# ZPP-Robotics/OSQP-Solver

Hardware: AMD Instinct MI355X
Metric: QPs/sec on a 1024-QP batch of box-QPs (n=512, m=1024), OSQP defaults; ADMM iters/sec alongside (higher is better)
Workload: dtype f64

## Files before the change

### include/mi_osqp.h

```cpp
#ifndef MI_OSQP_H
#define MI_OSQP_H

#include <stdint.h>

#ifdef __cplusplus
extern "C" {
#endif

typedef enum {
  MI_OSQP_OK = 0,
  MI_OSQP_ERR_INVALID_DATA = 1,
  MI_OSQP_ERR_INVALID_SETTINGS = 2,
  MI_OSQP_ERR_PATTERN_CHANGED = 3,
  MI_OSQP_ERR_NONCONVEX = 4,
  MI_OSQP_ERR_DEVICE = 5,
  MI_OSQP_ERR_NULL = 6,
  MI_OSQP_ERR_ALLOC = 7
} mi_osqp_error;

typedef enum {
  MI_OSQP_EXIT_OPTIMAL = 0,
  MI_OSQP_EXIT_PRIMAL_INFEASIBLE = 1,
  MI_OSQP_EXIT_DUAL_INFEASIBLE = 2,
  MI_OSQP_EXIT_OPTIMAL_INACCURATE = 3,
  MI_OSQP_EXIT_PRIMAL_INFEASIBLE_INACCURATE = 4,
  MI_OSQP_EXIT_DUAL_INFEASIBLE_INACCURATE = 5,
  MI_OSQP_EXIT_MAX_ITERATIONS = 6,
  MI_OSQP_EXIT_INTERRUPTED = 7,
  MI_OSQP_EXIT_TIME_LIMIT_REACHED = 8,
  MI_OSQP_EXIT_NON_CONVEX = 9,
  MI_OSQP_EXIT_UNKNOWN = 10
} mi_osqp_exit_code;

typedef struct {
  double  rho;
  double  sigma;
  int64_t scaling;
  int64_t adaptive_rho;
  int64_t adaptive_rho_interval;
  double  adaptive_rho_tolerance;
  int64_t max_iter;
  double  eps_abs;
  double  eps_rel;
  double  eps_prim_inf;
  double  eps_dual_inf;
  double  alpha;
  int64_t scaled_termination;
  int64_t check_termination;
  int64_t warm_start;
  int64_t verbose;
  int64_t polish;
  int64_t polish_refine_iter;
  double  delta;
} mi_osqp_settings;

typedef struct {
  int64_t iter;
  int64_t status_val;
  int64_t exit_code;
  double  obj_val;
  double  pri_res;
  double  dua_res;
  int64_t rho_updates;
  double  rho_estimate;
  double  rho;
  int64_t status_polish;
} mi_osqp_info;

typedef struct {
  int64_t n, m, N, batch, tile, n_tiles;
  int64_t nnz_P_triu, nnz_A, nnz_KKT, nnz_L;
  int64_t n_supernodes, n_blocks;
  int64_t fwd_levels, bwd_levels, fwd_slots, bwd_slots, chk_slots;
  int64_t lds_bytes, threads_per_block;
  int64_t dense_tail_rows, dense_tail_slots;
  double  setup_seconds_host, setup_seconds_factor, setup_seconds_upload;
  int64_t nnz_L_before_tail;
  int64_t solve_groups, solve_group_threads;
  int64_t resident_state, lds_bytes_iterate;
  int64_t pipelined_refactors;
  int64_t resident_factor_steps, lds_bytes_factor;
  int64_t dense_tail_tasks, dense_tail_waves_used, dense_tail_wave_tasks_max;
  int64_t refactor_lanes;
  int64_t iterate_launches_deep_ring, iterate_launches_long_head;
  int64_t runahead_regions, runahead_tiles, runahead_left, runahead_missed;
} mi_osqp_stats;

typedef struct mi_osqp_solver mi_osqp_solver;
typedef struct mi_osqp_batch  mi_osqp_batch;

void        mi_osqp_default_settings(mi_osqp_settings *s);
const char *mi_osqp_exit_code_name(int64_t exit_code);
const char *mi_osqp_error_name(int64_t err);
const char *mi_osqp_version(void);
const char *mi_osqp_last_error(void);

int mi_osqp_setup(mi_osqp_solver **out, int64_t n, int64_t m,
                  const int64_t *P_colptr, const int64_t *P_rowidx, const double *P_val,
                  const double *q,
                  const int64_t *A_colptr, const int64_t *A_rowidx, const double *A_val,
                  const double *l, const double *u, const mi_osqp_settings *settings);
int mi_osqp_update_A(mi_osqp_solver *h, const int64_t *A_colptr, const int64_t *A_rowidx,
                     const double *A_val);
int mi_osqp_update_bounds(mi_osqp_solver *h, const double *l, const double *u);
int mi_osqp_update_A_bounds(mi_osqp_solver *h, const int64_t *A_colptr, const int64_t *A_rowidx, const double *A_val,
                            const double *l, const double *u);
int mi_osqp_warm_start_x(mi_osqp_solver *h, const double *x);
int mi_osqp_update_q(mi_osqp_solver *h, const double *q);
int mi_osqp_update_P(mi_osqp_solver *h, const int64_t *P_colptr, const int64_t *P_rowidx, const double *P_val);
int mi_osqp_update_P_A(mi_osqp_solver *h, const int64_t *P_colptr, const int64_t *P_rowidx, const double *P_val,
                       const int64_t *A_colptr, const int64_t *A_rowidx, const double *A_val);
int mi_osqp_warm_start_y(mi_osqp_solver *h, const double *y);
int mi_osqp_solve(mi_osqp_solver *h, mi_osqp_info *info);
int mi_osqp_get_primal(mi_osqp_solver *h, double *x_out);
int mi_osqp_get_dual(mi_osqp_solver *h, double *y_out);
int mi_osqp_get_prim_inf_cert(mi_osqp_solver *h, double *dy_out );
int mi_osqp_get_dual_inf_cert(mi_osqp_solver *h, double *dx_out );
int mi_osqp_adjoint(mi_osqp_solver *h, const double *dx, const double *dy, double *dq, double *dP, double *dA, double *dl, double *du,
                    int32_t *status);
int mi_osqp_get_stats(mi_osqp_solver *h, mi_osqp_stats *st);
int mi_osqp_get_settings(mi_osqp_solver *h, mi_osqp_settings *out);
int mi_osqp_update_settings(mi_osqp_solver *h, const mi_osqp_settings *s);
void mi_osqp_free(mi_osqp_solver *h);

int mi_osqp_batch_setup(mi_osqp_batch **out, int64_t B, int64_t n, int64_t m,
                        const int64_t *P_colptr, const int64_t *P_rowidx, const double *P_val,
                        const double *q,
                        const int64_t *A_colptr, const int64_t *A_rowidx, const double *A_val,
                        const double *l, const double *u, const mi_osqp_settings *settings,
                        int64_t device);
int mi_osqp_batch_update_A(mi_osqp_batch *h, const int64_t *A_colptr, const int64_t *A_rowidx,
                           const double *A_val);
int mi_osqp_batch_update_bounds(mi_osqp_batch *h, const double *l, const double *u);
int mi_osqp_batch_update_A_bounds(mi_osqp_batch *h, const int64_t *A_colptr, const int64_t *A_rowidx, const double *A_val,
                                  const double *l, const double *u);
int mi_osqp_batch_warm_start_x(mi_osqp_batch *h, const double *x);
int mi_osqp_batch_update_q(mi_osqp_batch *h, const double *q);
int mi_osqp_batch_update_P(mi_osqp_batch *h, const int64_t *P_colptr, const int64_t *P_rowidx, const double *P_val);
int mi_osqp_batch_update_P_A(mi_osqp_batch *h, const int64_t *P_colptr, const int64_t *P_rowidx, const double *P_val,
                             const int64_t *A_colptr, const int64_t *A_rowidx, const double *A_val);
int mi_osqp_batch_warm_start_y(mi_osqp_batch *h, const double *y);
int mi_osqp_batch_get_P_upper_pattern(mi_osqp_batch *h, int64_t *colptr, int64_t *rowidx, int64_t *nnz_out);
int mi_osqp_batch_solve(mi_osqp_batch *h);
int mi_osqp_batch_get_primal(mi_osqp_batch *h, double *x_out );
int mi_osqp_batch_get_dual(mi_osqp_batch *h, double *y_out );
int mi_osqp_batch_get_info(mi_osqp_batch *h, mi_osqp_info *info );
int mi_osqp_batch_get_prim_inf_cert(mi_osqp_batch *h, double *dy_out );
int mi_osqp_batch_get_dual_inf_cert(mi_osqp_batch *h, double *dx_out );
int mi_osqp_batch_get_stats(mi_osqp_batch *h, mi_osqp_stats *st);
int mi_osqp_batch_get_ordering(mi_osqp_batch *h, int64_t *kkt_perm);
void mi_osqp_batch_free(mi_osqp_batch *h);
int mi_osqp_prefetch_analysis(int64_t B, int64_t n, int64_t m, const int64_t *Pp, const int64_t *Pi,
                              const int64_t *Ap, const int64_t *Ai, int64_t device);
void mi_osqp_release_device_cache(void);

int mi_osqp_batch_update_bounds_device(mi_osqp_batch *h, const double *d_l, const double *d_u, void *stream);
int mi_osqp_batch_update_A_bounds_device(mi_osqp_batch *h, const double *d_Av, const double *d_l, const double *d_u, void *stream);
int mi_osqp_batch_update_q_device(mi_osqp_batch *h, const double *d_q, void *stream);
int mi_osqp_batch_update_P_device(mi_osqp_batch *h, const double *d_Pv, void *stream);
int mi_osqp_batch_update_P_A_bounds_device(mi_osqp_batch *h, const double *d_Pv, const double *d_Av, const double *d_l, const double *d_u,
                                           void *stream);
int mi_osqp_batch_solve_device(mi_osqp_batch *h, double *d_x_out, int32_t *d_status, int32_t *d_iters, void *stream);
int mi_osqp_batch_reset(mi_osqp_batch *h);
int mi_osqp_batch_last_solve_stats(mi_osqp_batch *h, int64_t *total_iters, int64_t *kernel_launches,
                                   double *device_seconds, double *refactor_seconds, int64_t *refactor_count,
                                   double *compact_seconds);
int mi_osqp_batch_last_polish_stats(mi_osqp_batch *h, int64_t *polished, int64_t *accepted, double *seconds);
int mi_osqp_batch_get_polish_active(mi_osqp_batch *h, int8_t *act);
// ... 40 lines not shown
  MI_GOMP_MODEL_DH_CHAIN = 6
} mi_gomp_model;
typedef struct { int32_t model; int32_t is_gripper; double radius; double param[12]; } mi_gomp_ball;
typedef struct { double dir[2]; double point[3]; int32_t below; int32_t reserved; } mi_gomp_line;
typedef struct mi_gomp_scene mi_gomp_scene;
int mi_gomp_scene_create(mi_gomp_scene **out, mi_osqp_batch *h, int64_t dims, int64_t waypoints,
                         int64_t n_balls, const mi_gomp_ball *balls, int64_t n_lines, const mi_gomp_line *lines,
                         const double *con_lo, const double *con_hi);
typedef struct { int32_t n_joints; int32_t reserved; double a[8], d[8], alpha[8], theta0[8]; } mi_gomp_chain;
int mi_gomp_scene_create_chain(mi_gomp_scene **out, mi_osqp_batch *h, int64_t dims, int64_t waypoints,
                               const mi_gomp_chain *chain, int64_t n_balls, const mi_gomp_ball *balls,
                               int64_t n_lines, const mi_gomp_line *lines, const double *con_lo, const double *con_hi);
typedef struct { double a[3], b[3]; double radius; double margin; } mi_gomp_capsule;
int mi_gomp_scene_create_world(mi_gomp_scene **out, mi_osqp_batch *h, int64_t dims, int64_t waypoints,
                               const mi_gomp_chain *chain, int64_t n_balls, const mi_gomp_ball *balls,
                               int64_t n_lines, const mi_gomp_line *lines, int64_t n_capsules, const mi_gomp_capsule *capsules,
                               const double *con_lo, const double *con_hi);
void mi_gomp_scene_free(mi_gomp_scene *sc);
int mi_gomp_scene_set_rows(mi_gomp_scene *sc, int64_t n_ids, const int64_t *ids, const double *A_val, const double *l, const double *u);
int mi_gomp_scene_get_rows(mi_gomp_scene *sc, int64_t id, double *A_val, double *l, double *u);
int mi_gomp_assemble_some(mi_gomp_scene *sc, int64_t n_ids, const int64_t *ids, const double *x, int32_t *ok_out);
int mi_gomp_relinearise_some(mi_gomp_scene *sc, int64_t n_ids, const int64_t *ids, const double *x, int32_t *ok_out);

typedef struct mi_osqp_multi mi_osqp_multi;
int mi_osqp_multi_batch_setup(mi_osqp_multi **out, int64_t n_devices, const int64_t *devices,
                              int64_t B, int64_t n, int64_t m,
                              const int64_t *P_colptr, const int64_t *P_rowidx, const double *P_val,
                              const double *q,
                              const int64_t *A_colptr, const int64_t *A_rowidx, const double *A_val,
                              const double *l, const double *u, const mi_osqp_settings *settings);
int mi_osqp_multi_batch_update_A(mi_osqp_multi *h, const int64_t *A_colptr, const int64_t *A_rowidx, const double *A_val);
int mi_osqp_multi_batch_update_bounds(mi_osqp_multi *h, const double *l, const double *u);
int mi_osqp_multi_batch_update_A_bounds(mi_osqp_multi *h, const int64_t *A_colptr, const int64_t *A_rowidx, const double *A_val,
                                        const double *l, const double *u);
int mi_osqp_multi_batch_warm_start_x(mi_osqp_multi *h, const double *x);
int mi_osqp_multi_batch_update_q(mi_osqp_multi *h, const double *q);
int mi_osqp_multi_batch_update_P(mi_osqp_multi *h, const int64_t *P_colptr, const int64_t *P_rowidx, const double *P_val);
int mi_osqp_multi_batch_update_P_A(mi_osqp_multi *h, const int64_t *P_colptr, const int64_t *P_rowidx, const double *P_val,
                                   const int64_t *A_colptr, const int64_t *A_rowidx, const double *A_val);
int mi_osqp_multi_batch_warm_start_y(mi_osqp_multi *h, const double *y);
int mi_osqp_multi_batch_get_settings(mi_osqp_multi *h, mi_osqp_settings *out);
int mi_osqp_multi_batch_update_settings(mi_osqp_multi *h, const mi_osqp_settings *s);
int mi_osqp_multi_batch_update_rho_each(mi_osqp_multi *h, const double *rho );
int mi_osqp_multi_batch_solve(mi_osqp_multi *h);
int mi_osqp_multi_batch_solve_async(mi_osqp_multi *h);
int mi_osqp_multi_batch_wait(mi_osqp_multi *h);
int mi_osqp_multi_batch_get_primal(mi_osqp_multi *h, double *x_out );
int mi_osqp_multi_batch_get_dual(mi_osqp_multi *h, double *y_out );
int mi_osqp_multi_batch_get_info(mi_osqp_multi *h, mi_osqp_info *info );
int mi_osqp_multi_batch_get_prim_inf_cert(mi_osqp_multi *h, double *dy_out );
int mi_osqp_multi_batch_get_dual_inf_cert(mi_osqp_multi *h, double *dx_out );
int64_t mi_osqp_multi_batch_shards(mi_osqp_multi *h);
int mi_osqp_multi_batch_shard(mi_osqp_multi *h, int64_t k, int64_t *device, int64_t *begin, int64_t *end, mi_osqp_batch **handle);
void mi_osqp_multi_batch_free(mi_osqp_multi *h);

int mi_osqp_batch_spmv(mi_osqp_batch *h, const double *d_x, const double *d_y,
                       double *d_Px, double *d_Aty, double *d_Ax, void *stream);
int mi_osqp_batch_kkt_solve(mi_osqp_batch *h, const double *d_rhs, double *d_sol, void *stream);
int mi_osqp_batch_refactor_device(mi_osqp_batch *h);
int mi_osqp_batch_kernel_time(mi_osqp_batch *h, double *avg_ms, int64_t *launches);
int mi_osqp_batch_refactor_time(mi_osqp_batch *h, double *factor_ms, double *tail_ms, int64_t *launches, int64_t *qps);
int mi_osqp_batch_refactor_peak(mi_osqp_batch *h, int64_t *qps, double *factor_ms, double *tail_ms);

int mi_osqp_batch_get_scaling(mi_osqp_batch *h, double *D , double *E , double *c );

int mi_osqp_debug_host_kkt_solve(int64_t n, int64_t m,
                                 const int64_t *P_colptr, const int64_t *P_rowidx, const double *P_val,
                                 const int64_t *A_colptr, const int64_t *A_rowidx, const double *A_val,
                                 const double *l, const double *u, const mi_osqp_settings *settings,
                                 int64_t tile, const double *rhs ,
                                 double *sol_schedule , double *sol_direct ,
                                 mi_osqp_stats *st);

int mi_osqp_debug_host_block_factor(int64_t n, int64_t m,
                                    const int64_t *P_colptr, const int64_t *P_rowidx, const double *P_val,
                                    const int64_t *A_colptr, const int64_t *A_rowidx, const double *A_val,
                                    const double *l, const double *u, const mi_osqp_settings *settings,
                                    double *max_rel_diff_L, double *max_rel_diff_Dinv, int64_t *counts);

int mi_osqp_debug_refactor_chunks(int64_t n_flagged, const int64_t *flagged, int64_t n_active, const int64_t *active, int64_t tile,
                                  int64_t chunk_qps, int64_t max_chunks, int64_t *n_chunks, int64_t *work_begin, int64_t *tiles,
                                  int64_t *tile_begin);

int mi_osqp_debug_refactor_lanes(int64_t n_flagged, const int64_t *flagged, int64_t n_active, const int64_t *active, int64_t tile,
                                 int64_t chunk_qps, int64_t max_chunks, int64_t kbt, int64_t lanes, int64_t chunk0_first,
                                 int64_t scratch_slots, int64_t *n_lanes, int64_t *lane_of, int64_t *order, int64_t *order_begin,
                                 int64_t *scratch_begin, int64_t *n_waits, int64_t *wait_chunk, int64_t *wait_for);

int mi_osqp_debug_runahead_group(int64_t n_active, const int64_t *tiles, const double *pri_res, const double *dua_res, int64_t size,
                                 int64_t min_active, int64_t *n_group, int64_t *group);

int mi_osqp_debug_iterate_form(int64_t tiles, int64_t has_head, int64_t forced_form, int64_t long_min, int64_t *form);

int mi_osqp_debug_trace_kkt_solve(mi_osqp_batch *h, int32_t which, const double *d_rhs, double *d_sol,
                                  uint32_t *out, int64_t out_capacity_words, int64_t *dims);

#ifdef __cplusplus
}
#endif
#endif
```

### osqp-solver_amd/__init__.py

```python
import ctypes as C
import os

import numpy as np

try:
    import torch
except ImportError:
    torch = None

from . import build as _build

_HERE = os.path.dirname(os.path.abspath(__file__))
_LIB = None

EXIT_NAMES = ["kOptimal", "kPrimalInfeasible", "kDualInfeasible", "kOptimalInaccurate",
              "kPrimalInfeasibleInaccurate", "kDualInfeasibleInaccurate", "kMaxIterations",
              "kInterrupted", "kTimeLimitReached", "kNonConvex", "kUnknown"]
K_OPTIMAL = 0


class Settings(C.Structure):
    _fields_ = [("rho", C.c_double), ("sigma", C.c_double), ("scaling", C.c_int64),
                ("adaptive_rho", C.c_int64), ("adaptive_rho_interval", C.c_int64),
                ("adaptive_rho_tolerance", C.c_double), ("max_iter", C.c_int64),
                ("eps_abs", C.c_double), ("eps_rel", C.c_double), ("eps_prim_inf", C.c_double),
                ("eps_dual_inf", C.c_double), ("alpha", C.c_double), ("scaled_termination", C.c_int64),
                ("check_termination", C.c_int64), ("warm_start", C.c_int64), ("verbose", C.c_int64),
                ("polish", C.c_int64), ("polish_refine_iter", C.c_int64), ("delta", C.c_double)]


class Info(C.Structure):
    _fields_ = [("iter", C.c_int64), ("status_val", C.c_int64), ("exit_code", C.c_int64),
                ("obj_val", C.c_double), ("pri_res", C.c_double), ("dua_res", C.c_double),
                ("rho_updates", C.c_int64), ("rho_estimate", C.c_double), ("rho", C.c_double),
                ("status_polish", C.c_int64)]

    def as_dict(self):
        return {k: getattr(self, k) for k, _ in self._fields_}


class Stats(C.Structure):
    _fields_ = [(k, C.c_int64) for k in
                ("n", "m", "N", "batch", "tile", "n_tiles", "nnz_P_triu", "nnz_A", "nnz_KKT", "nnz_L",
                 "n_supernodes", "n_blocks", "fwd_levels", "bwd_levels", "fwd_slots", "bwd_slots",
                 "chk_slots", "lds_bytes", "threads_per_block", "dense_tail_rows", "dense_tail_slots")] + \
               [(k, C.c_double) for k in ("setup_seconds_host", "setup_seconds_factor", "setup_seconds_upload")] + \
               [("nnz_L_before_tail", C.c_int64), ("solve_groups", C.c_int64), ("solve_group_threads", C.c_int64),
                ("resident_state", C.c_int64), ("lds_bytes_iterate", C.c_int64), ("pipelined_refactors", C.c_int64),
                ("resident_factor_steps", C.c_int64), ("lds_bytes_factor", C.c_int64),
                ("dense_tail_tasks", C.c_int64), ("dense_tail_waves_used", C.c_int64), ("dense_tail_wave_tasks_max", C.c_int64),
                ("refactor_lanes", C.c_int64),
                ("iterate_launches_deep_ring", C.c_int64), ("iterate_launches_long_head", C.c_int64),
                ("runahead_regions", C.c_int64), ("runahead_tiles", C.c_int64), ("runahead_left", C.c_int64),
                ("runahead_missed", C.c_int64)]

    def as_dict(self):
        return {k: getattr(self, k) for k, _ in self._fields_}


class MiOsqpError(RuntimeError):
    def __init__(self, code, where):
        self.code = int(code)
        L = lib()
        msg = L.mi_osqp_error_name(int(code)).decode()
        extra = L.mi_osqp_last_error().decode()
        super().__init__(f"{where}: error {int(code)} ({msg}) {extra}")


def lib():
    global _LIB
    if _LIB is None:
        path = os.path.join(_HERE, "libmi_osqp.so")
        if os.environ.get("MI_OSQP_LIBRARY"):
            path = os.environ["MI_OSQP_LIBRARY"]
        else:
            try:
                path = _build.build()
            except Exception as e:
                if not os.path.exists(path):
                    raise ImportError(f"libmi_osqp.so missing and could not be built: {e}") from e
        L = C.CDLL(path)
        ip, dp, vp = C.POINTER(C.c_int64), C.POINTER(C.c_double), C.c_void_p
        L.mi_osqp_default_settings.argtypes = [C.POINTER(Settings)]
        for f in ("mi_osqp_exit_code_name", "mi_osqp_error_name"):
            getattr(L, f).restype = C.c_char_p; getattr(L, f).argtypes = [C.c_int64]
        L.mi_osqp_version.restype = C.c_char_p
        L.mi_osqp_last_error.restype = C.c_char_p
        L.mi_osqp_batch_setup.argtypes = [C.POINTER(vp), C.c_int64, C.c_int64, C.c_int64, ip, ip, dp, dp, ip, ip, dp,
                                          dp, dp, C.POINTER(Settings), C.c_int64]
        L.mi_osqp_batch_update_A.argtypes = [vp, ip, ip, dp]
        L.mi_osqp_batch_update_A_bounds.argtypes = [vp, ip, ip, dp, dp, dp]
        L.mi_osqp_batch_update_bounds.argtypes = [vp, dp, dp]
        L.mi_osqp_batch_warm_start_x.argtypes = [vp, dp]
        L.mi_osqp_batch_update_q.argtypes = [vp, dp]
        L.mi_osqp_batch_update_q_device.argtypes = [vp, vp, vp]
        L.mi_osqp_batch_update_P.argtypes = [vp, ip, ip, dp]
        L.mi_osqp_batch_update_P_A.argtypes = [vp, ip, ip, dp, ip, ip, dp]
        L.mi_osqp_batch_warm_start_y.argtypes = [vp, dp]
        L.mi_osqp_batch_get_P_upper_pattern.argtypes = [vp, ip, ip, ip]
        L.mi_osqp_batch_update_P_device.argtypes = [vp, vp, vp]
        L.mi_osqp_batch_update_P_A_bounds_device.argtypes = [vp, vp, vp, vp, vp, vp]
        L.mi_osqp_batch_update_P_some.argtypes = [vp, C.c_int64, ip, dp]
        L.mi_osqp_batch_update_P_A_bounds_some.argtypes = [vp, C.c_int64, ip, dp, dp, dp, dp]
        L.mi_osqp_batch_update_q_some.argtypes = [vp, C.c_int64, ip, dp]
        L.mi_osqp_batch_warm_start_y_some.argtypes = [vp, C.c_int64, ip, dp]
        L.mi_osqp_settings_update_check.argtypes = [C.POINTER(Settings), C.POINTER(Settings)]
        L.mi_osqp_batch_get_settings.argtypes = [vp, C.POINTER(Settings)]
        L.mi_osqp_batch_update_settings.argtypes = [vp, C.POINTER(Settings)]
        L.mi_osqp_batch_update_rho_each.argtypes = [vp, dp]
        L.mi_osqp_batch_update_rho_some.argtypes = [vp, C.c_int64, ip, dp]
        L.mi_osqp_get_settings.argtypes = [vp, C.POINTER(Settings)]
        L.mi_osqp_update_settings.argtypes = [vp, C.POINTER(Settings)]
        L.mi_osqp_multi_batch_get_settings.argtypes = [vp, C.POINTER(Settings)]
        L.mi_osqp_multi_batch_update_settings.argtypes = [vp, C.POINTER(Settings)]
        L.mi_osqp_multi_batch_update_rho_each.argtypes = [vp, dp]
        L.mi_osqp_batch_solve.argtypes = [vp]
        L.mi_osqp_batch_get_primal.argtypes = [vp, dp]
        L.mi_osqp_batch_get_dual.argtypes = [vp, dp]
        L.mi_osqp_batch_get_info.argtypes = [vp, C.POINTER(Info)]
        for f in ("mi_osqp_get_prim_inf_cert", "mi_osqp_get_dual_inf_cert", "mi_osqp_batch_get_prim_inf_cert",
                  "mi_osqp_batch_get_dual_inf_cert", "mi_osqp_multi_batch_get_prim_inf_cert", "mi_osqp_multi_batch_get_dual_inf_cert"):
            getattr(L, f).argtypes = [vp, dp]
        L.mi_osqp_batch_get_prim_inf_cert_some.argtypes = [vp, C.c_int64, ip, dp]
        L.mi_osqp_batch_get_dual_inf_cert_some.argtypes = [vp, C.c_int64, ip, dp]
        L.mi_osqp_batch_get_stats.argtypes = [vp, C.POINTER(Stats)]
        L.mi_osqp_batch_get_ordering.argtypes = [vp, ip]
        L.mi_osqp_batch_free.argtypes = [vp]; L.mi_osqp_batch_free.restype = None
        L.mi_osqp_batch_update_bounds_device.argtypes = [vp, vp, vp, vp]
        L.mi_osqp_batch_update_A_bounds_device.argtypes = [vp, vp, vp, vp, vp]
        L.mi_osqp_batch_solve_device.argtypes = [vp, vp, vp, vp, vp]
        L.mi_osqp_batch_reset.argtypes = [vp]
        L.mi_osqp_batch_refactor_device.argtypes = [vp]
        L.mi_osqp_batch_last_solve_stats.argtypes = [vp, ip, ip, dp, dp, ip, dp]
        L.mi_osqp_batch_last_polish_stats.argtypes = [vp, ip, ip, dp]
        L.mi_osqp_batch_get_polish_active.argtypes = [vp, C.POINTER(C.c_int8)]
        L.mi_osqp_batch_adjoint.argtypes = [vp, dp, dp, dp, dp, dp, dp, dp, C.POINTER(C.c_int32)]
        L.mi_osqp_adjoint.argtypes = [vp, dp, dp, dp, dp, dp, dp, dp, C.POINTER(C.c_int32)]
        L.mi_osqp_batch_adjoint_device.argtypes = [vp] * 10
        L.mi_osqp_batch_get_scaling.argtypes = [vp, dp, dp, dp]
        L.mi_osqp_batch_spmv.argtypes = [vp, vp, vp, vp, vp, vp, vp]
        L.mi_osqp_batch_kkt_solve.argtypes = [vp, vp, vp, vp]
        L.mi_osqp_batch_kernel_time.argtypes = [vp, dp, ip]
        L.mi_osqp_batch_refactor_time.argtypes = [vp, dp, dp, ip, ip]
        L.mi_osqp_batch_refactor_peak.argtypes = [vp, ip, dp, dp]
        L.mi_osqp_batch_reinit_some.argtypes = [vp, C.c_int64, ip, dp, dp, dp]
        L.mi_osqp_batch_update_A_bounds_some.argtypes = [vp, C.c_int64, ip, dp, dp, dp]
        L.mi_osqp_batch_warm_start_x_some.argtypes = [vp, C.c_int64, ip, dp]
        L.mi_osqp_batch_solve_begin_some.argtypes = [vp, C.c_int64, ip]
        L.mi_osqp_batch_polish_some.argtypes = [vp, C.c_int64, ip]
        L.mi_osqp_batch_advance.argtypes = [vp, C.c_int64]
        L.mi_osqp_batch_poll.argtypes = [vp, C.c_int64, ip, ip, C.c_int64]
        L.mi_osqp_batch_get_primal_some.argtypes = [vp, C.c_int64, ip, dp]
        L.mi_osqp_batch_get_dual_some.argtypes = [vp, C.c_int64, ip, dp]
        L.mi_osqp_batch_get_info_some.argtypes = [vp, C.c_int64, ip, C.POINTER(Info)]
        L.mi_osqp_batch_running.argtypes = [vp]; L.mi_osqp_batch_running.restype = C.c_int64
        L.mi_osqp_batch_ring_wraps.argtypes = [vp]; L.mi_osqp_batch_ring_wraps.restype = C.c_int64
        L.mi_osqp_release_device_cache.argtypes = []; L.mi_osqp_release_device_cache.restype = None
        L.mi_osqp_setup.argtypes = [C.POINTER(vp), C.c_int64, C.c_int64, ip, ip, dp, dp, ip, ip, dp, dp, dp, C.POINTER(Settings)]
        L.mi_osqp_update_A.argtypes = [vp, ip, ip, dp]
        L.mi_osqp_update_bounds.argtypes = [vp, dp, dp]
        L.mi_osqp_warm_start_x.argtypes = [vp, dp]
        L.mi_osqp_update_q.argtypes = [vp, dp]
        L.mi_osqp_update_P.argtypes = [vp, ip, ip, dp]
        L.mi_osqp_update_P_A.argtypes = [vp, ip, ip, dp, ip, ip, dp]
        L.mi_osqp_warm_start_y.argtypes = [vp, dp]
        L.mi_osqp_solve.argtypes = [vp, C.POINTER(Info)]
        L.mi_osqp_get_primal.argtypes = [vp, dp]
        L.mi_osqp_get_dual.argtypes = [vp, dp]
        L.mi_osqp_get_stats.argtypes = [vp, C.POINTER(Stats)]
        L.mi_osqp_free.argtypes = [vp]; L.mi_osqp_free.restype = None
        L.mi_osqp_multi_batch_setup.argtypes = [C.POINTER(vp), C.c_int64, ip, C.c_int64, C.c_int64, C.c_int64, ip, ip, dp, dp,
                                                ip, ip, dp, dp, dp, C.POINTER(Settings)]
        L.mi_osqp_multi_batch_update_A.argtypes = [vp, ip, ip, dp]
        L.mi_osqp_multi_batch_update_bounds.argtypes = [vp, dp, dp]
        L.mi_osqp_multi_batch_update_A_bounds.argtypes = [vp, ip, ip, dp, dp, dp]
        L.mi_osqp_multi_batch_warm_start_x.argtypes = [vp, dp]
        L.mi_osqp_multi_batch_update_q.argtypes = [vp, dp]
        L.mi_osqp_multi_batch_update_P.argtypes = [vp, ip, ip, dp]
        L.mi_osqp_multi_batch_update_P_A.argtypes = [vp, ip, ip, dp, ip, ip, dp]
        L.mi_osqp_multi_batch_warm_start_y.argtypes = [vp, dp]
        L.mi_osqp_multi_batch_solve.argtypes = [vp]
        L.mi_osqp_multi_batch_solve_async.argtypes = [vp]
        L.mi_osqp_multi_batch_wait.argtypes = [vp]
        L.mi_osqp_multi_batch_get_primal.argtypes = [vp, dp]
        L.mi_osqp_multi_batch_get_dual.argtypes = [vp, dp]
        L.mi_osqp_multi_batch_get_info.argtypes = [vp, C.POINTER(Info)]
        L.mi_osqp_multi_batch_shards.argtypes = [vp]; L.mi_osqp_multi_batch_shards.restype = C.c_int64
        L.mi_osqp_multi_batch_shard.argtypes = [vp, C.c_int64, ip, ip, ip, C.POINTER(vp)]
        L.mi_osqp_multi_batch_free.argtypes = [vp]; L.mi_osqp_multi_batch_free.restype = None
        L.mi_osqp_debug_host_kkt_solve.argtypes = [C.c_int64, C.c_int64, ip, ip, dp, ip, ip, dp, dp, dp,
                                                   C.POINTER(Settings), C.c_int64, dp, dp, dp, C.POINTER(Stats)]
        L.mi_osqp_debug_refactor_chunks.argtypes = [C.c_int64, ip, C.c_int64, ip, C.c_int64, C.c_int64, C.c_int64, ip, ip, ip, ip]
        L.mi_osqp_debug_refactor_lanes.argtypes = [C.c_int64, ip, C.c_int64, ip] + [C.c_int64] * 7 + [ip] * 8
        L.mi_osqp_debug_runahead_group.argtypes = [C.c_int64, ip, dp, dp, C.c_int64, C.c_int64, ip, ip]
        L.mi_osqp_debug_iterate_form.argtypes = [C.c_int64] * 4 + [ip]
        L.mi_osqp_prefetch_analysis.argtypes = [C.c_int64, C.c_int64, C.c_int64, ip, ip, ip, ip, C.c_int64]
        L.mi_osqp_debug_host_block_factor.argtypes = [C.c_int64, C.c_int64, ip, ip, dp, ip, ip, dp, dp, dp,
                                                      C.POINTER(Settings), dp, dp, ip]
        _LIB = L
    return _LIB


def host_cores():
    try:
        n = len(os.sched_getaffinity(0))
    except Exception:
        n = os.cpu_count() or 1
    for path in ("/sys/fs/cgroup/cpu.max",):
        try:
            quota, period = open(path).read().split()[:2]
            if quota != "max":
                n = min(n, max(1, int(round(int(quota) / int(period)))))
        except Exception:
            pass
    try:
        q = int(open("/sys/fs/cgroup/cpu/cpu.cfs_quota_us").read())
        p = int(open("/sys/fs/cgroup/cpu/cpu.cfs_period_us").read())
        if q > 0:
            n = min(n, max(1, int(round(q / p))))
    except Exception:
        pass
    return n


def default_settings(**kw):
    s = Settings()
    lib().mi_osqp_default_settings(C.byref(s))
    for k, v in kw.items():
        if not hasattr(s, k):
            raise KeyError(k)
        setattr(s, k, v)
    return s


class HandleSettings(Settings):

    def bind(self, getter):
        self._getter = getter
        return self

    def __call__(self):
        out = Settings()
        self._getter(out)
        C.memmove(C.byref(self), C.byref(out), C.sizeof(Settings))
        return out


def settings_update_check(in_force, wanted):
    return int(lib().mi_osqp_settings_update_check(C.byref(in_force), C.byref(wanted)))


def _handle_settings(kw, get_name, owner):
    import weakref
    hs = HandleSettings()
    C.memmove(C.byref(hs), C.byref(default_settings(**kw)), C.sizeof(Settings))
    ref = weakref.ref(owner)

    def getter(out):
        _chk(getattr(lib(), get_name)(ref()._h, C.byref(out)), get_name)
    return hs.bind(getter)


def _update_settings(self, fn_name, fields):
    s = self.settings()
    for k, v in fields.items():
        if not hasattr(s, k):
            raise KeyError(k)
        setattr(s, k, v)
    _chk(getattr(lib(), fn_name)(self._h, C.byref(s)), fn_name)
    return self.settings()


def _i64(a):
    return np.ascontiguousarray(a, dtype=np.int64)


def _f64(a):
# ... 498 lines not shown
        return self._b.update_settings(**fields)

    def solve(self):
        info = self._b.solve()[0]
        return int(info.exit_code), self._b.primal()[0]

    def info(self):
        return self._b.info()[0]

    def dual(self):
        return self._b.dual()[0]

    def prim_inf_cert(self):
        return self._b.prim_inf_cert()[0]

    def dual_inf_cert(self):
        return self._b.dual_inf_cert()[0]

    def adjoint(self, dx, dy=None):
        out = self._b.adjoint(dx, dy)
        return {k: (int(v[0]) if k == "status" else v[0]) for k, v in out.items()}

    def stats(self):
        return self._b.stats()


def debug_host_kkt_solve(P, A, l, u, rhs, tri_waves=0, **settings):
    L = lib()
    P, A = _csc(P), _csc(A)
    n, m = A.shape[1], A.shape[0]
    s = default_settings(**settings)
    rhs = _f64(rhs)
    sol_s, sol_d = np.empty(n + m), np.empty(n + m)
    st = Stats()
    Pp, Pi, Px = _i64(P.indptr), _i64(P.indices), _f64(P.data)
    Ap, Ai, Ax = _i64(A.indptr), _i64(A.indices), _f64(A.data)
    l, u = _f64(l), _f64(u)
    rc = L.mi_osqp_debug_host_kkt_solve(n, m, _ip(Pp), _ip(Pi), _dp(Px), _ip(Ap), _ip(Ai), _dp(Ax), _dp(l), _dp(u),
                                        C.byref(s), 1 + int(tri_waves), _dp(rhs), _dp(sol_s), _dp(sol_d), C.byref(st))
    _chk(rc, "debug_host_kkt_solve")
    return sol_s, sol_d, st.as_dict()


def prefetch_analysis(P, A, B=1, device=-1, check=True):
    L = lib()
    P, A = _csc(P), _csc(A)
    n, m = A.shape[1], A.shape[0]
    Pp, Pi, Ap, Ai = _i64(P.indptr), _i64(P.indices), _i64(A.indptr), _i64(A.indices)
    rc = L.mi_osqp_prefetch_analysis(B, n, m, _ip(Pp), _ip(Pi), _ip(Ap), _ip(Ai), device)
    if check:
        _chk(rc, "prefetch_analysis")
    return rc


def debug_refactor_chunks(flagged, active, tile, chunk_qps, max_chunks=8):
    f, a = _i64(flagged), _i64(active)
    nch = C.c_int64()
    wb = np.zeros(max_chunks + 2, dtype=np.int64); tb = np.zeros(max_chunks + 2, dtype=np.int64)
    tl = np.zeros(max(1, len(a)), dtype=np.int64)
    _chk(lib().mi_osqp_debug_refactor_chunks(len(f), _ip(f), len(a), _ip(a), tile, chunk_qps, max_chunks, C.byref(nch), _ip(wb), _ip(tl),
                                             _ip(tb)), "debug_refactor_chunks")
    k = int(nch.value)
    return ([f[wb[c]:wb[c + 1]].tolist() for c in range(k)], [tl[tb[c]:tb[c + 1]].tolist() for c in range(k)])


def debug_refactor_lanes(flagged, active, tile, chunk_qps, lanes, kbt=None, chunk0_first=False, scratch_slots=None, max_chunks=8):
    f, a = _i64(flagged), _i64(active)
    kbt = tile if kbt is None else kbt
    work, _ = debug_refactor_chunks(flagged, active, tile, chunk_qps, max_chunks)
    k = len(work)
    nl, nw = C.c_int64(), C.c_int64()
    lane_of = np.zeros(max_chunks + 2, dtype=np.int64); order = np.zeros(max_chunks + 2, dtype=np.int64)
    ob = np.zeros(4, dtype=np.int64); sb = np.zeros(max_chunks + 2, dtype=np.int64)
    wc = np.zeros((max_chunks + 1) ** 2, dtype=np.int64); wf = np.zeros((max_chunks + 1) ** 2, dtype=np.int64)
    _chk(lib().mi_osqp_debug_refactor_lanes(len(f), _ip(f), len(a), _ip(a), tile, chunk_qps, max_chunks, kbt, lanes, int(bool(chunk0_first)),
                                            2 ** 31 - 1 if scratch_slots is None else scratch_slots, C.byref(nl), _ip(lane_of), _ip(order),
                                            _ip(ob), _ip(sb), C.byref(nw), _ip(wc), _ip(wf)), "debug_refactor_lanes")
    L = int(nl.value)
    return dict(n_lanes=L, lane_of=lane_of[:k].tolist(), order=[order[ob[l]:ob[l + 1]].tolist() for l in range(L)],
                scratch=[(int(sb[c]), (len(work[c]) + kbt - 1) // kbt * kbt) for c in range(k)],
                waits=list(zip(wc[:nw.value].tolist(), wf[:nw.value].tolist())))


def debug_runahead_group(tiles, pri_res, dua_res, size, min_active):
    t, p, d = _i64(tiles), _f64(pri_res), _f64(dua_res)
    if not (len(t) == len(p) == len(d)):
        raise ValueError("tiles, pri_res and dua_res differ in length")
    ng = C.c_int64()
    out = np.zeros(max(1, len(t)), dtype=np.int64)
    _chk(lib().mi_osqp_debug_runahead_group(len(t), _ip(t), _dp(p), _dp(d), size, min_active, C.byref(ng), _ip(out)), "debug_runahead_group")
    return out[:ng.value].tolist()


def debug_iterate_form(tiles, has_head=True, forced_form=0, long_min=-1):
    form = C.c_int64()
    _chk(lib().mi_osqp_debug_iterate_form(tiles, int(bool(has_head)), forced_form, long_min, C.byref(form)), "debug_iterate_form")
    return int(form.value)


def debug_host_block_factor(P, A, l, u, **settings):
    L = lib()
    P, A = _csc(P), _csc(A)
    n, m = A.shape[1], A.shape[0]
    s = default_settings(**settings)
    Pp, Pi, Px = _i64(P.indptr), _i64(P.indices), _f64(P.data)
    Ap, Ai, Ax = _i64(A.indptr), _i64(A.indices), _f64(A.data)
    l, u = _f64(l), _f64(u)
    dL, dD = C.c_double(), C.c_double()
    cnt = (C.c_int64 * 4)()
    rc = L.mi_osqp_debug_host_block_factor(n, m, _ip(Pp), _ip(Pi), _dp(Px), _ip(Ap), _ip(Ai), _dp(Ax), _dp(l), _dp(u),
                                           C.byref(s), C.byref(dL), C.byref(dD), cnt)
    _chk(rc, "debug_host_block_factor")
    return dL.value, dD.value, dict(blocks=cnt[0], triples=cnt[1], storage=cnt[2], levels=cnt[3])
```

### osqp-solver_amd/csrc/host_core.cpp

```cpp
#include "host_core.hpp"
#include "sched_format.h"

#include <algorithm>
#include <cmath>
#include <cstdio>
#include <cstdlib>
#include <cstring>
#include <limits>
#include <numeric>
#include <set>
#include <chrono>
#include <thread>

#include "../../include/mi_osqp.h"

namespace miosqp {

int validate_settings(const Settings &s) {
  if (s.scaling < 0 || s.max_iter <= 0 || s.check_termination < 0) return 1;
  if (s.adaptive_rho != 0 && s.adaptive_rho != 1) return 1;
  if (s.adaptive_rho_interval < 0 || s.adaptive_rho_tolerance < 1.0) return 1;
  if (!(s.rho > 0.0) || !(s.sigma > 0.0)) return 1;
  if (s.eps_abs < 0.0 || s.eps_rel < 0.0 || (s.eps_abs == 0.0 && s.eps_rel == 0.0)) return 1;
  if (!(s.eps_prim_inf > 0.0) || !(s.eps_dual_inf > 0.0)) return 1;
// ... 844 lines not shown
    }
    dt.n_lt = (int)dt.lt_pos.size(); dt.n_ltcol = (int)dt.ltcol_col.size();
    const uint16_t zero_slot = (uint16_t)dt.n_lt;
    for (auto &fr : frag) for (auto &f : fr) for (uint16_t &v : f.second) if (v == 0xFFFFu) v = zero_slot;
    struct TileRec { int I, J; std::vector<std::pair<int, int>> src; };
    std::vector<TileRec> tiles;
    for (int I = 0; I < nt; I++)
      for (int J = 0; J <= I; J++) {
        TileRec t{I, J, {}};
        size_t a = 0, b = 0;
        while (a < frag[I].size() && b < frag[J].size()) {
          if (frag[I][a].first < frag[J][b].first) a++;
          else if (frag[I][a].first > frag[J][b].first) b++;
          else { t.src.push_back({(int)a, (int)b}); a++; b++; }
        }
        tiles.push_back(std::move(t));
      }
    const int nw = 16;
    std::vector<int> order(tiles.size());
    std::iota(order.begin(), order.end(), 0);
    std::stable_sort(order.begin(), order.end(), [&](int x, int y) { return tiles[x].src.size() > tiles[y].src.size(); });
    std::vector<std::vector<int>> mine(nw);
    for (size_t d = 0; d < order.size(); d++) { const size_t round = d / nw, pos = d % nw; mine[(round & 1) ? nw - 1 - pos : pos].push_back(order[d]); }
    dt.tile_tab.clear(); dt.wave_tiles.assign(nw + 1, 0u); dt.asm_q.clear(); dt.asm_qcol.clear();
    for (int w = 0; w < nw; w++) {
      dt.wave_tiles[w] = (uint32_t)(dt.tile_tab.size() / 4);
      for (int ti : mine[w]) {
        const TileRec &t = tiles[ti];
        const uint32_t q0 = (uint32_t)(dt.asm_q.size() / 64);
        const size_t padded = (t.src.size() + 31) / 32 * 32;
        for (size_t s0 = 0; s0 < padded; s0 += 4) {
          for (int g = 0; g < 4; g++) {
            const bool real = s0 + g < t.src.size();
            const auto *fa = real ? &frag[t.I][t.src[s0 + g].first] : nullptr;
            const auto *fb = real ? &frag[t.J][t.src[s0 + g].second] : nullptr;
            dt.asm_qcol.push_back(real ? (uint16_t)fa->first : (uint16_t)0);
            for (int e = 0; e < 16; e++) dt.asm_q.push_back(real ? ((uint32_t)fa->second[e] | ((uint32_t)fb->second[e] << 16)) : ((uint32_t)zero_slot | ((uint32_t)zero_slot << 16)));
          }
        }
        const uint32_t blk_id = find_blk(ct0 + t.I, ct0 + t.J);
        dt.tile_tab.insert(dt.tile_tab.end(), {((uint32_t)t.I << 16) | (uint32_t)t.J, bf.blk[4 * blk_id], q0, (uint32_t)(dt.asm_q.size() / 64)});
      }
    }
    dt.wave_tiles[nw] = (uint32_t)(dt.tile_tab.size() / 4);
    dt.asm_q64.resize(dt.asm_q.size());
    for (size_t e = 0; e < dt.asm_q.size(); e++) {
      const uint64_t w = dt.asm_q[e], ci = dt.asm_qcol[e / 16];
      dt.asm_q64[e] = ((w & 0xFFFFu) * 8u) | ((((w >> 16) * 8u) | ((ci * 8u) << 17)) << 32);
    }
    dt.src_tile.resize(dt.src.size());
    for (size_t e = 0; e < dt.src.size(); e++) {
      const int32_t sc = dt.src[e];
      dt.src_tile[e] = sc < 0 ? sc : (int32_t)dt_tile_offset(sc % k, sc / k);
    }
    dt.diag_tile.resize(k);
    for (int i = 0; i < k; i++) dt.diag_tile[i] = dt_tile_offset(i, i);
    dt.task_step.clear();
    { uint32_t pos = 0; for (size_t t = 0; t < dt.task.size() / 4; t++) { dt.task_step.push_back(pos); pos += dt.task[4 * t + 3]; } }
  }
}


Tuning tuning_from_env() {
  Tuning t;
  if (const char *e = getenv("MI_OSQP_TILE")) { const int v = atoi(e); if (v == 1 || v == 2 || v == 4) t.tile = v; }
  if (const char *e = getenv("MI_OSQP_THREADS")) t.threads = std::max(64, std::min(1024, atoi(e) / 64 * 64));
  t.global_xs = getenv("MI_OSQP_GLOBAL_XS") != nullptr;
  if (const char *e = getenv("MI_OSQP_GROUPS")) t.groups = std::max(0, std::min(256, atoi(e)));
  if (const char *e = getenv("MI_OSQP_GROUP_THREADS")) t.group_threads = std::max(64, std::min(512, atoi(e) / 64 * 64));
  if (const char *e = getenv("MI_OSQP_ASSUME_CUS")) t.assume_cus = std::max(0, atoi(e));
  if (const char *e = getenv("MI_OSQP_FACTOR_THREADS")) t.factor_threads = std::max(64, std::min(1024, atoi(e) / 64 * 64));
  if (const char *e = getenv("MI_OSQP_FACTOR_GROUPS")) t.factor_groups = std::max(1, std::min(256, atoi(e)));
  t.ruiz = getenv("MI_OSQP_HOST_RUIZ") ? 1 : getenv("MI_OSQP_DEVICE_RUIZ") ? -1 : 0;
  if (const char *e = getenv("MI_OSQP_CONT_RING_KB")) t.cont_ring_kb = std::max(0L, atol(e));
  if (const char *e = getenv("MI_OSQP_ANALYSIS_CACHE")) t.analysis_cache = atoi(e) != 0;
  t.stream_state = getenv("MI_OSQP_STREAM_STATE") != nullptr;
  t.stream_factor = getenv("MI_OSQP_STREAM_FACTOR") != nullptr;
  if (const char *e = getenv("MI_OSQP_REFACTOR_PIPELINE")) t.refactor_pipeline = atoi(e) != 0;
  if (const char *e = getenv("MI_OSQP_REFACTOR_PIPELINE_MIN")) t.pipeline_min = std::max(0, atoi(e));
  if (const char *e = getenv("MI_OSQP_REFACTOR_CHUNKS")) t.pipeline_chunks = std::max(0, std::min(8, atoi(e)));
  if (const char *e = getenv("MI_OSQP_REFACTOR_CHUNK_QPS")) t.pipeline_chunk_qps = std::max(0, atoi(e));
  if (const char *e = getenv("MI_OSQP_REFACTOR_LANES")) t.refactor_lanes = std::max(1, std::min(3, atoi(e)));
  if (const char *e = getenv("MI_OSQP_REFACTOR_CHUNK0")) t.lanes_chunk0 = atoi(e) != 0;
  if (const char *e = getenv("MI_OSQP_RUNAHEAD")) t.runahead = atoi(e) != 0;
  if (const char *e = getenv("MI_OSQP_RUNAHEAD_TILES")) t.runahead_tiles = std::max(0, atoi(e));
  if (const char *e = getenv("MI_OSQP_RUNAHEAD_MIN")) t.runahead_min = std::max(0, atoi(e));
  if (const char *e = getenv("MI_OSQP_RUNAHEAD_END")) t.runahead_end = std::max(0, atoi(e));
  if (const char *e = getenv("MI_OSQP_RF_FORM")) { const int v = atoi(e); if (v == kIterDeepRing || v == kIterLongHead) t.rf_form = v; }
  if (const char *e = getenv("MI_OSQP_RF_LONG_MIN")) t.rf_long_min = std::max(0, atoi(e));
  AnalysisTuning &a = t.analysis;
  if (const char *e = getenv("MI_OSQP_DENSE_TAIL")) a.dense_tail = atoi(e);
  if (const char *e = getenv("MI_OSQP_ORDERING")) a.ordering = e[0];
  if (const char *e = getenv("MI_OSQP_ND_LEAF")) a.nd_leaf = atoi(e);
  if (const char *e = getenv("MI_OSQP_RELAX")) a.relax = atoi(e);
  a.serial = getenv("MI_OSQP_SERIAL_ANALYSIS") != nullptr;
  return t;
}

RefactorChunks refactor_chunks(const std::vector<int> &flagged, const std::vector<int> &active, int bt, int chunk_qps, int max_chunks) {
  RefactorChunks rc;
  const int nq = (int)flagged.size();
  max_chunks = std::max(1, max_chunks);
  chunk_qps = std::max(1, chunk_qps);
  if ((nq + chunk_qps - 1) / chunk_qps > max_chunks) chunk_qps = (nq + max_chunks - 1) / max_chunks;
  const int n_ref = (nq + chunk_qps - 1) / chunk_qps;
  rc.n_chunks = 1 + n_ref;
  rc.work_begin.assign(1, 0);
  for (int c = 0; c <= n_ref; c++) rc.work_begin.push_back(std::min(nq, c * chunk_qps));
  std::vector<std::pair<int, int>> tc;
  size_t f = 0;
  for (size_t i = 0; i < active.size(); i++) {
    const int tile = active[i] / bt;
    if (i && active[i - 1] / bt == tile) continue;
    int chunk = 0;
    while (f < flagged.size() && flagged[f] / bt < tile) f++;
    for (size_t g = f; g < flagged.size() && flagged[g] / bt == tile; g++) chunk = 1 + (int)g / chunk_qps;
    tc.emplace_back(chunk, tile);
  }
  std::stable_sort(tc.begin(), tc.end(), [](const std::pair<int, int> &x, const std::pair<int, int> &y) { return x.first < y.first; });
  rc.tile_begin.assign((size_t)rc.n_chunks + 1, 0);
  for (const auto &p : tc) { rc.tiles.push_back(p.second); rc.tile_begin[(size_t)p.first + 1]++; }
  for (int c = 0; c < rc.n_chunks; c++) rc.tile_begin[(size_t)c + 1] += rc.tile_begin[c];
  return rc;
}

RefactorLanes refactor_lanes(const RefactorChunks &ch, const std::vector<int> &flagged, int bt, int kbt, int lanes, bool chunk0_first, int scratch_slots) {
  RefactorLanes rl;
  const int nc = ch.n_chunks, n_ref = nc - 1;
  bt = std::max(1, bt); kbt = std::max(1, kbt);
  int L = std::max(1, std::min(std::min(3, lanes), std::max(1, n_ref)));
  std::vector<int> padded((size_t)nc + 1, 0);
  for (int c = 1; c < nc; c++) padded[(size_t)c + 1] = padded[c] + (ch.work_begin[(size_t)c + 1] - ch.work_begin[c] + kbt - 1) / kbt * kbt;
  if (padded[nc] > scratch_slots) L = 1;
  rl.n_lanes = L;
  rl.lane_of.assign(nc, 0);
  rl.order.assign(L, std::vector<int>());
  rl.scratch_begin.assign((size_t)nc + 1, 0);
  if (L == 1) {
    for (int c = 0; c < nc; c++) rl.order[0].push_back(c);
    return rl;
  }
  rl.scratch_begin = padded;
  for (int c = 1; c < nc; c++) { rl.lane_of[c] = (c - 1) % L; rl.order[(c - 1) % L].push_back(c); }
  if (chunk0_first) { rl.lane_of[0] = L - 1; rl.order[L - 1].insert(rl.order[L - 1].begin(), 0); }
  else {
    int at = L - 1;
    for (int a = L - 1; a >= 0; a--) if (rl.order[a].size() < rl.order[at].size()) at = a;
    rl.lane_of[0] = at; rl.order[at].push_back(0);
  }
  for (int c = 1; c < nc; c++) {
    std::vector<char> need(nc, 0);
    for (int t = ch.tile_begin[c]; t < ch.tile_begin[(size_t)c + 1]; t++) {
      const int tile = ch.tiles[t];
      size_t g = std::lower_bound(flagged.begin(), flagged.end(), tile * bt) - flagged.begin();
      for (; g < flagged.size() && flagged[g] / bt == tile; g++) {
        const int d = (int)(std::upper_bound(ch.work_begin.begin() + 1, ch.work_begin.end(), (int)g) - ch.work_begin.begin()) - 1;
        if (d >= 1 && d < c && rl.lane_of[d] != rl.lane_of[c]) need[d] = 1;
      }
    }
    for (int d = 1; d < c; d++) if (need[d]) { rl.wait_chunk.push_back(c); rl.wait_for.push_back(d); }
  }
  return rl;
}

std::vector<int> runahead_group(const std::vector<int> &tiles, const std::vector<double> &pri, const std::vector<double> &dua, int size, int min_active) {
  const size_t na = tiles.size();
  if (!na || size <= 0 || na < (size_t)std::max(0, min_active) || pri.size() != na || dua.size() != na) return {};
  const double inf = std::numeric_limits<double>::infinity();
  auto scaled = [&](const std::vector<double> &r) {
    std::vector<double> v(na);
    for (size_t i = 0; i < na; i++) v[i] = std::isnan(r[i]) ? inf : r[i];
    std::vector<double> s = v;
    std::nth_element(s.begin(), s.begin() + na / 2, s.end());
    const double med = s[na / 2];
    for (size_t i = 0; i < na; i++) v[i] = v[i] == inf ? inf : med == inf ? 0.0 : med > 0.0 ? v[i] / med : v[i] > 0.0 ? inf : 0.0;
    return v;
  };
  const std::vector<double> sp = scaled(pri), sd = scaled(dua);
  std::vector<std::pair<double, int>> order(na);
  for (size_t i = 0; i < na; i++) order[i] = {sp[i] + sd[i], tiles[i]};
  std::sort(order.begin(), order.end(), [](const std::pair<double, int> &x, const std::pair<double, int> &y) {
    return x.first > y.first || (x.first == y.first && x.second < y.second);
  });
  std::vector<int> group(std::min(na, (size_t)size));
  for (size_t i = 0; i < group.size(); i++) group[i] = order[i].second;
  return group;
}

int iterate_form(int tiles, bool has_head, const Tuning &t) {
  if (!has_head) return kIterStreamed;
  if (t.rf_form == kIterDeepRing || t.rf_form == kIterLongHead) return t.rf_form;
  const int long_min = t.rf_long_min >= 0 ? t.rf_long_min : kRfLongMinDefault;
  return tiles > 0 && tiles >= long_min ? kIterLongHead : kIterDeepRing;
}


int analyze(int64_t n64, int64_t m64, const int64_t *Pp, const int64_t *Pi, const int64_t *Ap,
            const int64_t *Ai, const AnalysisTuning &tune, Analysis &an, int nwaves, int bt, int max_extra_rows, int dense_tail_max, int tri_waves, int n_tiles) {
  if (nwaves < 1 || nwaves > 16 || (bt != 1 && bt != 2 && bt != 4) || tri_waves < 0 || tri_waves > 2048) return MI_OSQP_ERR_INVALID_SETTINGS;
  if (n64 <= 0 || m64 < 0 || !Pp || !Ap || n64 + m64 > (int64_t)1 << 30) return MI_OSQP_ERR_INVALID_DATA;
  int n = (int)n64, m = (int)m64, N = n + m;
  an = Analysis();
  an.n = n; an.m = m; an.N = N;
  if (Pp[0] != 0 || Ap[0] != 0) return MI_OSQP_ERR_INVALID_DATA;
  for (int j = 0; j < n; j++) {
    if (Pp[j + 1] < Pp[j] || Ap[j + 1] < Ap[j]) return MI_OSQP_ERR_INVALID_DATA;
// ... 782 lines not shown
```

### osqp-solver_amd/csrc/host_core.hpp

```cpp
#pragma once

#include <cstdint>
#include <string>
#include <vector>

namespace miosqp {

constexpr double kInfty = 1e30;
constexpr double kRhoMin = 1e-6, kRhoMax = 1e6, kRhoEqOverIneq = 1e3, kRhoTol = 1e-4;
constexpr double kMinScaling = 1e-4, kMaxScaling = 1e4;
constexpr double kDivisionTol = 1.0 / kInfty;
constexpr int kChunk = 16;
constexpr uint32_t kNoRow = 0xFFFFFFFFu;

struct Settings {
  double rho = 0.1, sigma = 1e-6;
  int64_t scaling = 10, adaptive_rho = 1, adaptive_rho_interval = 0;
  double adaptive_rho_tolerance = 5.0;
  int64_t max_iter = 4000;
  double eps_abs = 1e-3, eps_rel = 1e-3, eps_prim_inf = 1e-4, eps_dual_inf = 1e-4, alpha = 1.6;
  int64_t scaled_termination = 0, check_termination = 25, warm_start = 1, verbose = 0;
  int64_t polish = 0, polish_refine_iter = 3;
  double delta = 1e-6;
};
int validate_settings(const Settings &s);

struct AnalysisTuning {
  int dense_tail = -1;
  char ordering = 0;
  int nd_leaf = 0;
  int relax = -1;
  bool serial = false;
  bool operator==(const AnalysisTuning &o) const {
    return dense_tail == o.dense_tail && ordering == o.ordering && nd_leaf == o.nd_leaf && relax == o.relax && serial == o.serial;
  }
};
constexpr bool kRunaheadDefault = true;
struct Tuning {
  int tile = 0;
  int threads = 0;
  bool global_xs = false;
  int groups = -1;
  int group_threads = 0;
  int assume_cus = 0;
  int factor_threads = 1024;
  int factor_groups = 0;
  int ruiz = 0;
  long cont_ring_kb = -1;
  bool analysis_cache = true;
  bool stream_state = false;
  bool stream_factor = false;
  bool refactor_pipeline = true;
  int pipeline_min = 0;
  int pipeline_chunks = 0;
  int pipeline_chunk_qps = 0;
  int refactor_lanes = 0;
  int lanes_chunk0 = -1;
  bool runahead = kRunaheadDefault;
  int runahead_tiles = 0;
  int runahead_min = 0;
  int runahead_end = 0;
  int rf_form = 0;
  int rf_long_min = -1;
  AnalysisTuning analysis;
};
Tuning tuning_from_env();

enum IterateForm { kIterStreamed = 0, kIterDeepRing = 1, kIterLongHead = 2 };
constexpr int kRfLongMinDefault = 0;
int iterate_form(int tiles, bool has_head, const Tuning &t);

struct RefactorChunks {
  int n_chunks = 1;
  std::vector<int> work_begin;
  std::vector<int> tiles;
  std::vector<int> tile_begin;
};
RefactorChunks refactor_chunks(const std::vector<int> &flagged, const std::vector<int> &active, int bt, int chunk_qps, int max_chunks);

struct RefactorLanes {
  int n_lanes = 1;
  std::vector<int> lane_of;
  std::vector<std::vector<int>> order;
  std::vector<int> scratch_begin;
  std::vector<int> wait_chunk, wait_for;
};
RefactorLanes refactor_lanes(const RefactorChunks &ch, const std::vector<int> &flagged, int bt, int kbt, int lanes, bool chunk0_first, int scratch_slots);

std::vector<int> runahead_group(const std::vector<int> &tiles, const std::vector<double> &pri, const std::vector<double> &dua, int size, int min_active);

struct Schedule {
  int n_phases = 0, nw = 0, bt = 1;
  bool barriers = true;
  std::vector<uint32_t> phase;
  std::vector<int> level_first_phase;
  std::vector<uint32_t> step;
  std::vector<uint32_t> step_ob;
  std::vector<uint32_t> outA;
  std::vector<uint32_t> idx;
  std::vector<uint32_t> idxw;
  std::vector<uint64_t> idxw64;
  std::vector<int32_t> src;
  uint32_t n_slots = 0;
  uint32_t n_steps = 0;
  std::vector<uint32_t> wave_range;
  std::vector<uint32_t> lvl_pos;
  std::vector<uint32_t> tail_bar;
  bool dataflow = false;
  uint32_t shadow = 0, pad = 0;
  uint32_t phys_steps() const { return n_steps; }
  size_t phase_stride() const { return 4 * (size_t)nw + 1; }
  int n_levels = 0;
};

struct BlockFactor {
  uint32_t storage = 0;
  std::vector<uint32_t> blk;
  std::vector<uint32_t> lvl;
  std::vector<uint32_t> utask;
  std::vector<uint32_t> tri;
  std::vector<uint32_t> tri4;
  std::vector<uint32_t> utask4;
  bool overflow = false;
  std::vector<uint32_t> ubig;
  std::vector<uint32_t> dtask4;
  std::vector<uint32_t> ttask4;
  std::vector<uint32_t> dtask;
  std::vector<uint32_t> ttask;
  std::vector<uint32_t> asm_dst;
  std::vector<uint32_t> asm_src;
  std::vector<int32_t> lpos;
  int n_levels = 0;
  size_t n_blocks() const { return blk.size() / 4; }
};
enum { ASM_P = 0, ASM_P_SIGMA = 1, ASM_SIGMA = 2, ASM_A = 3, ASM_NEG_RHOINV = 4 };

struct DenseTail {
  int s = 0, k = 0, nb = 0;
  int nw = 0, n_phases = 0;
  uint32_t n_steps = 0;
  std::vector<uint32_t> task;
  std::vector<uint32_t> wave_task;
  std::vector<uint32_t> wave_step;
  std::vector<uint32_t> tail_bar;
  std::vector<int32_t> src;
  std::vector<uint32_t> sblk;
  int n_lt = 0, n_ltcol = 0;
  std::vector<uint32_t> lt_pos;
  std::vector<uint32_t> ltcol_col;
  std::vector<uint32_t> tile_tab;
  std::vector<uint32_t> wave_tiles;
  std::vector<uint32_t> asm_q;
  std::vector<uint16_t> asm_qcol;
  std::vector<uint64_t> asm_q64;
  std::vector<int32_t> src_tile;
  std::vector<uint32_t> diag_tile;
  std::vector<uint32_t> task_step;
  size_t asm_lds_bytes() const { return ((size_t)n_lt + 1 + (size_t)n_ltcol) * sizeof(double); }
};
inline uint32_t dt_tile_offset(int i, int j) {
  const int I = i / 16, J = j / 16, r = i % 16, c = j % 16;
// ... 76 lines not shown
```

### osqp-solver_amd/csrc/solver.hip

```cpp
#include <hip/hip_runtime.h>
#include <time.h>

#include <algorithm>
#include <atomic>
#include <chrono>
#include <cmath>
#include <condition_variable>
#include <functional>
#include <limits>
#include <cstdio>
#include <cstdlib>
#include <cstring>
#include <string>
#include <thread>
#include <map>
#include <memory>
#include <mutex>
#include <vector>

#include "../../include/mi_osqp.h"
#include "device_types.h"
#include "host_core.hpp"

using namespace miosqp;
// ... 64 lines not shown
    }
    long long q1 = -1, p1 = 0;
    if (FILE *f = fopen("/sys/fs/cgroup/cpu/cpu.cfs_quota_us", "r")) { if (fscanf(f, "%lld", &q1) != 1) q1 = -1; fclose(f); }
    if (FILE *f = fopen("/sys/fs/cgroup/cpu/cpu.cfs_period_us", "r")) { if (fscanf(f, "%lld", &p1) != 1) p1 = 0; fclose(f); }
    if (q1 > 0 && p1 > 0) t = std::min<long long>(t, std::max<long long>(1, (q1 + p1 / 2) / p1));
  }
  cached = std::max(1, std::min(t, 128));
  return cached;
}

template <class F>
static void parallel_for(int count, F &&fn) {
  int nt = std::min(host_threads(), count);
  if (nt <= 1) { for (int i = 0; i < count; i++) fn(i, 0); return; }
  std::atomic<int> next{0};
  std::vector<std::thread> th;
  for (int t = 0; t < nt; t++)
    th.emplace_back([&, t]() { for (int i; (i = next.fetch_add(1)) < count;) fn(i, t); });
  for (auto &x : th) x.join();
}

namespace devpool {
static std::mutex mu;
static std::multimap<std::pair<int, size_t>, void *> blocks;
static size_t kept = 0;
constexpr size_t kMaxKept = (size_t)8 << 30;
static void *take(int dev, size_t bytes, size_t &cap) {
  std::lock_guard<std::mutex> lk(mu);
  auto it = blocks.lower_bound({dev, bytes});
  if (it == blocks.end() || it->first.first != dev || it->first.second > 2 * bytes + 4096) return nullptr;
  void *p = it->second; cap = it->first.second; kept -= cap;
  blocks.erase(it);
  return p;
}
static bool give(int dev, void *p, size_t cap) {
  std::lock_guard<std::mutex> lk(mu);
  if (kept + cap > kMaxKept) return false;
  blocks.emplace(std::make_pair(dev, cap), p); kept += cap;
  return true;
}
static void release_all() {
  std::lock_guard<std::mutex> lk(mu);
  for (auto &b : blocks) (void)hipFree(b.second);
  blocks.clear(); kept = 0;
}
}

namespace hostpool {
static std::mutex mu;
static std::multimap<size_t, void *> blocks;
static size_t kept = 0;
constexpr size_t kMaxKept = (size_t)1 << 30;
static void *take(size_t bytes, size_t &cap) {
  std::lock_guard<std::mutex> lk(mu);
  auto it = blocks.lower_bound(bytes);
  if (it == blocks.end() || it->first > 4 * bytes + 65536) return nullptr;
  void *p = it->second; cap = it->first; kept -= cap;
  blocks.erase(it);
  return p;
}
static void give(void *p, size_t cap) {
  if (!p) return;
  {
    std::lock_guard<std::mutex> lk(mu);
    if (kept + cap <= kMaxKept) { blocks.emplace(cap, p); kept += cap; return; }
  }
  (void)hipHostFree(p);
}
static void release_all() {
  std::lock_guard<std::mutex> lk(mu);
  for (auto &b : blocks) (void)hipHostFree(b.second);
  blocks.clear(); kept = 0;
}
static hipError_t alloc(void **p, size_t bytes, size_t *cap) {
  bytes = (bytes + 4095) & ~(size_t)4095;
  if (void *q = take(bytes, *cap)) { *p = q; return hipSuccess; }
  *cap = bytes;
  return hipHostMalloc(p, bytes, hipHostMallocPortable);
}
}
namespace streampool {
constexpr int kPipeChunks = 8;
constexpr int kPipeLanes = 3;
constexpr int kPipeEvents = 3 + 3 * kPipeChunks + kPipeLanes;
struct Bundle { int dev; hipStream_t stream; hipEvent_t ev[5]; hipStream_t pipe_r, pipe_i, pipe_x; hipEvent_t pipe_ev[kPipeEvents]; };
static void destroy(const Bundle &b) {
  for (hipEvent_t e : b.ev) if (e) (void)hipEventDestroy(e);
  for (hipEvent_t e : b.pipe_ev) if (e) (void)hipEventDestroy(e);
  for (hipStream_t st : {b.stream, b.pipe_r, b.pipe_i, b.pipe_x}) if (st) (void)hipStreamDestroy(st);
}
static std::mutex mu;
static std::vector<Bundle> idle;
static bool take(int dev, Bundle &out) {
  std::lock_guard<std::mutex> lk(mu);
  for (size_t i = 0; i < idle.size(); i++)
    if (idle[i].dev == dev) { out = idle[i]; idle.erase(idle.begin() + i); return true; }
  return false;
}
static void give(const Bundle &b) {
  {
    std::lock_guard<std::mutex> lk(mu);
    if (idle.size() < 64) { idle.push_back(b); return; }
  }
  destroy(b);
}
static void release_all() {
  std::lock_guard<std::mutex> lk(mu);
  for (Bundle &b : idle) destroy(b);
  idle.clear();
}
}

template <class T>
struct DevBuf {
  T *p = nullptr; size_t n = 0;
  size_t cap = 0;
  int dev = 0;
  int alloc(size_t count) {
    free();
    n = count;
    if (!count) return 0;
    const size_t bytes = (count * sizeof(T) + 255) & ~(size_t)255;
    if (hipGetDevice(&dev) != hipSuccess) dev = 0;
    if (void *q = devpool::take(dev, bytes, cap)) { p = (T *)q; return 0; }
    hipError_t e = hipMalloc((void **)&p, bytes);
    if (e != hipSuccess) {
      devpool::release_all();
      e = hipMalloc((void **)&p, bytes);
    }
    if (e != hipSuccess) { p = nullptr; g_last_error = std::string("hipMalloc: ") + hipGetErrorString(e); return MI_OSQP_ERR_ALLOC; }
    cap = bytes;
    return 0;
  }
  int zero(hipStream_t s) { if (n && hipMemsetAsync(p, 0, n * sizeof(T), s) != hipSuccess) return MI_OSQP_ERR_DEVICE; return 0; }
  int upload(const std::vector<T> &v) {
    int rc = alloc(v.size());
    if (rc) return rc;
    if (v.size() && hipMemcpy(p, v.data(), v.size() * sizeof(T), hipMemcpyHostToDevice) != hipSuccess) return MI_OSQP_ERR_DEVICE;
    return 0;
  }
  void free() { if (p && !devpool::give(dev, p, cap)) (void)hipFree(p); p = nullptr; n = 0; cap = 0; }
  ~DevBuf() { free(); }
};

struct SchedBufs {
  DevBuf<uint32_t> step, idxw, lvl_pos, tail_bar;
  DevBuf<uint64_t> idxw64;
  DevBuf<int32_t> src;
  int upload(const Schedule &s) {
    int rc;
    if ((rc = step.upload(s.step)) || (rc = idxw.upload(s.idxw)) || (rc = idxw64.upload(s.idxw64)) || (rc = src.upload(s.src)) ||
        (rc = lvl_pos.upload(s.lvl_pos)) || (rc = tail_bar.upload(s.tail_bar))) return rc;
    return 0;
  }
  SchedDev view(const Schedule &s) const {
    SchedDev d; d.step = step.p; d.idxw = idxw.p; d.idxw64 = idxw64.p; d.lvl_pos = lvl_pos.p; d.tail_bar = tail_bar.p;
    d.n_phases = s.n_phases; d.nw = s.nw; d.n_levels = s.n_levels;
    d.n_steps = s.n_steps; d.n_slots = s.n_slots;
    return d;
  }
};

struct mi_osqp_batch {
  Settings st;
  bool rho_interval_auto = false;
  Tuning tune;
  std::shared_ptr<const Analysis> anp;
  int B = 0, BT = 1, ntiles = 0, threads = 512, device = 0, n_cus = 256;
  size_t lds = 0;
  size_t lds_iter = 0;
  int rs_off = 0;
  size_t lds_factor = 0;
  int rf_off = 0, rf_steps = 0;
  int64_t rf_launches[3] = {0, 0, 0};
  std::vector<QPNumeric> qp;
  bool host_bounds_stale = false;
  hipStream_t stream = nullptr;
  SchedBufs fwd, bwd, chk;
  DevBuf<uint32_t> pinv, xloc;
  DevBuf<double> fwd_val, bwd_val, chk_val, dinv, x, z, y, q, l, u, rho_vec, rho_inv, Dsc, Dsc_inv, Esc, Esc_inv;
  DevBuf<double> dx, dy, out1, out2, dscal, x_out, y_out, xs_global;
  DevBuf<double> cert_out;
  bool global_xs = false;
  int mw_groups = 0, mw_threads = 0;
  DevBuf<uint32_t> mw_bar;
  DevBuf<unsigned char> rflag;
  DevBuf<double> mw_scratch;
  DevBuf<double> fwd_val0, bwd_val0, dinv0, rho_vec0, rho_inv0, dscal0;
  DevBuf<int> use_work;
  DevBuf<int> iscal, flag, npos;
  DevBuf<uint32_t> bf_blk, bf_lvl, bf_utask, bf_tri, bf_dtask, bf_ttask, bf_asm_dst, bf_asm_src, bf_ubig;
  DevBuf<int32_t> fwd_srcblk, bwd_srcblk;
  DevBuf<double> pa_val, Lblk, Dl, dinv_scratch;
  DevBuf<uint32_t> dt_task, dt_wave_task, dt_wave_step, dt_tail_bar;
  DevBuf<uint32_t> dt_lt_pos, dt_ltcol_col, dt_tile_tab, dt_wave_tiles, dt_diag_tile, dt_task_step;
  DevBuf<uint64_t> dt_asm_q64;
  DevBuf<int32_t> dt_src_tile;
  int dt_nh = 0; uint32_t dt_cs_doubles = 0; size_t dt_lds = 0, dt_lds_asm = 0;
  DevBuf<int32_t> dt_src;
  DevBuf<double> dt_val, dt_val0, dt_Sd;
  DevBuf<uint32_t> sp_ptr, sp_ent;
  DevBuf<uint32_t> sp_ell, sp_rowid;
  int sp_npass = 0;
  uint32_t sp_ell_off[4] = {0, 0, 0, 0}, sp_ell_k[4] = {0, 0, 0, 0};
  bool host_rho_stale = false;
  bool host_scaling_stale = false;
  DevBuf<int32_t> rz_prow, rz_pcol, rz_arow, rz_acol;
  bool clear_rho_updates = true;
  int *h_npos = nullptr;
  DevBuf<double> stage; DevBuf<int> ids, work;
  int *h_iscal = nullptr;
  double *h_dscal = nullptr;
  size_t h_iscal_cap = 0, h_dscal_cap = 0, h_npos_cap = 0, pin_cap = 0;
  double *pin = nullptr;
  size_t pin_n = 0;
  hipEvent_t ev0 = nullptr, ev1 = nullptr, evf0 = nullptr, evf1 = nullptr, evf2 = nullptr;
  hipStream_t pipe_r = nullptr, pipe_i = nullptr, pipe_x = nullptr;
  hipEvent_t pipe_ev[streampool::kPipeEvents] = {};
  DevBuf<int> tile_list;
  int64_t pipelined_refactors = 0;
  int64_t refactor_lanes = 0;
  DevBuf<int> ra_list;
  DevBuf<double> ra_res;
  double *h_res = nullptr; int *h_mark = nullptr;
  size_t h_res_cap = 0, h_mark_cap = 0;
  int64_t ra_regions = 0, ra_tiles = 0, ra_left = 0, ra_missed = 0;
  double factor_ms_sum = 0.0, dense_ms_sum = 0.0;
  int64_t refactor_launches = 0, refactor_qps = 0, peak_qps = 0;
  double peak_factor_ms = 0.0, peak_tail_ms = 0.0;
  mi_osqp_stats stats{};
  int64_t last_total_iters = 0, last_launches = 0, last_refactors = 0;
  double last_device_s = 0.0, last_refactor_s = 0.0, kernel_ms_sum = 0.0;
  int64_t kernel_launches = 0, kernel_qp_iters = 0;
  bool solved_once = false;
  std::vector<char> failed;
  DevBuf<int> fail_list;
  DevBuf<double> rawP, rawq;
  DevBuf<double> pol_fwd, pol_bwd, pol_dinv, pol_dt, pol_sol;
  DevBuf<signed char> pol_act;
  DevBuf<int> pol_stat;
  std::vector<int> pol_status;
  int64_t pol_count = 0, pol_accepted = 0;
  double pol_seconds = 0.0;
  hipEvent_t evp0 = nullptr, evp1 = nullptr;
  DevBuf<int> adj_stat;
  struct Cont {
    bool on = false;
    int L = 25;
    unsigned launch_seq = 0;
    DevBuf<unsigned> stop;
    int64_t adv_seq = 0, polled_seq = 0;
    std::vector<char> running, clear_rho;
    std::vector<mi_osqp_info> info;
    int n_running = 0;
    int *h_is[2] = {nullptr, nullptr}; double *h_ds[2] = {nullptr, nullptr}; size_t h_is_cap[2] = {0, 0}, h_ds_cap[2] = {0, 0};
    hipEvent_t ev[2] = {nullptr, nullptr}; int64_t seq_of[2] = {0, 0};
    double *xh = nullptr, *yh = nullptr; size_t xh_cap = 0, yh_cap = 0;
    double *ch = nullptr; size_t ch_cap = 0;
    std::vector<int> cert_status;
    char *ring_h = nullptr; size_t ring_cap = 0, ring_h_cap = 0, ring_head = 0;
    int64_t ring_wraps = 0;
    DevBuf<char> ring_d;
    DevBuf<int> work;
    hipEvent_t ev_adv = nullptr;
    std::vector<int> epoch;
    DevBuf<double> rz_scratch;
    double *keepA = nullptr, *keepl = nullptr, *keepu = nullptr;
    DevBuf<unsigned> counter;
    unsigned *h_done = nullptr; size_t h_done_cap = 0;
    std::vector<char> polishable, polishing;
    std::vector<int> pol_status;
    int *h_pstat = nullptr; size_t h_pstat_cap = 0;
  } cont;
  ~mi_osqp_batch() {
    DevGuard guard(device);
    if (stream) (void)hipStreamSynchronize(stream);
    for (int k = 0; k < 2; k++) { hostpool::give(cont.h_is[k], cont.h_is_cap[k]); hostpool::give(cont.h_ds[k], cont.h_ds_cap[k]); if (cont.ev[k]) (void)hipEventDestroy(cont.ev[k]); }
    hostpool::give(cont.xh, cont.xh_cap); hostpool::give(cont.yh, cont.yh_cap); hostpool::give(cont.ch, cont.ch_cap); hostpool::give(cont.ring_h, cont.ring_h_cap);
    if (cont.ev_adv) (void)hipEventDestroy(cont.ev_adv);
    if (evp0) (void)hipEventDestroy(evp0);
    if (evp1) (void)hipEventDestroy(evp1);
    hostpool::give(cont.h_done, cont.h_done_cap); hostpool::give(cont.h_pstat, cont.h_pstat_cap);
    hostpool::give(h_iscal, h_iscal_cap); hostpool::give(h_dscal, h_dscal_cap); hostpool::give(pin, pin_cap); hostpool::give(h_npos, h_npos_cap);
    hostpool::give(h_res, h_res_cap); hostpool::give(h_mark, h_mark_cap);
    if (pipe_r) (void)hipStreamSynchronize(pipe_r);
    if (pipe_i) (void)hipStreamSynchronize(pipe_i);
    if (pipe_x) (void)hipStreamSynchronize(pipe_x);
    streampool::Bundle sb{device, stream, {ev0, ev1, evf0, evf1, evf2}, pipe_r, pipe_i, pipe_x, {}};
    for (int k = 0; k < streampool::kPipeEvents; k++) sb.pipe_ev[k] = pipe_ev[k];
    if (stream && ev0 && ev1 && evf0 && evf1 && evf2) streampool::give(sb);
    else streampool::destroy(sb);
  }
};

struct mi_osqp_solver { mi_osqp_batch *b = nullptr; };


static Settings to_settings(const mi_osqp_settings *s) {
  Settings t;
  if (!s) return t;
  t.rho = s->rho; t.sigma = s->sigma; t.scaling = s->scaling; t.adaptive_rho = s->adaptive_rho;
  t.adaptive_rho_interval = s->adaptive_rho_interval; t.adaptive_rho_tolerance = s->adaptive_rho_tolerance;
  t.max_iter = s->max_iter; t.eps_abs = s->eps_abs; t.eps_rel = s->eps_rel; t.eps_prim_inf = s->eps_prim_inf;
  t.eps_dual_inf = s->eps_dual_inf; t.alpha = s->alpha; t.scaled_termination = s->scaled_termination;
  t.check_termination = s->check_termination; t.warm_start = s->warm_start; t.verbose = s->verbose;
  t.polish = s->polish; t.polish_refine_iter = s->polish_refine_iter; t.delta = s->delta;
  return t;
}

static void dense_tail_deal_stats(const DenseTail &dt, mi_osqp_stats &s) {
  s.dense_tail_tasks = s.dense_tail_waves_used = s.dense_tail_wave_tasks_max = 0;
  if (!dt.k) return;
  s.dense_tail_tasks = (int64_t)dt.task.size() / 4;
  for (int w = 0; w < dt.nw; w++) {
    const int64_t c = (int64_t)dt.wave_task[w + 1] - (int64_t)dt.wave_task[w];
    s.dense_tail_waves_used += c > 0; s.dense_tail_wave_tasks_max = std::max(s.dense_tail_wave_tasks_max, c);
  }
}

static size_t lds_bytes(int N, int BT, int threads) {
  int nw = threads / 64;
  return ((size_t)N * BT + (size_t)nw * 14 * BT + 14 * BT) * sizeof(double);
}

static KernelArgs make_args(mi_osqp_batch *h) {
  KernelArgs a{};
  a.n = (*h->anp).n; a.m = (*h->anp).m; a.N = (*h->anp).N; a.B = h->B;
  a.fwd = h->fwd.view((*h->anp).fwd); a.bwd = h->bwd.view((*h->anp).bwd); a.chk = h->chk.view((*h->anp).chk);
  a.pinv = h->pinv.p; a.xloc = h->xloc.p;
  a.fwd_val = h->fwd_val.p; a.bwd_val = h->bwd_val.p; a.chk_val = h->chk_val.p; a.dinv = h->dinv.p;
  a.fwd_val0 = h->fwd_val0.p; a.bwd_val0 = h->bwd_val0.p; a.dt_val0 = h->dt_val0.p;
  a.use_work = (h->fwd_val0.p && h->bwd_val0.p && (!(*h->anp).dt.k || h->dt_val0.p)) ? h->use_work.p : nullptr;
  a.x = h->x.p; a.z = h->z.p; a.y = h->y.p; a.q = h->q.p; a.l = h->l.p; a.u = h->u.p;
  a.rho_vec = h->rho_vec.p; a.rho_inv = h->rho_inv.p; a.Dsc = h->Dsc.p; a.Dsc_inv = h->Dsc_inv.p;
  a.Esc = h->Esc.p; a.Esc_inv = h->Esc_inv.p; a.dx = h->dx.p; a.dy = h->dy.p; a.out1 = h->out1.p; a.out2 = h->out2.p;
  a.dscal = h->dscal.p; a.iscal = h->iscal.p;
  a.x_out = h->x_out.p; a.y_out = h->y_out.p;
  a.cert_out = h->cert_out.p; a.cert_stride = (int)std::max<int64_t>(std::max<int64_t>(a.n, a.m), 1);
  a.xs_global = h->global_xs ? h->xs_global.p : nullptr; a.xs_len = (*h->anp).xs_total; a.wide = (*h->anp).wide ? 1 : 0;
  a.rs_off = h->rs_off; a.rf_off = h->rf_off;
  a.rf_form = iterate_form(h->ntiles, h->rf_off != 0, h->tune);
  a.mw_groups = h->mw_groups; a.mw_bar = h->mw_bar.p; a.mw_scratch = h->mw_scratch.p;
  a.df = (*h->anp).df ? 1 : 0; a.df_shadow = (unsigned)(*h->anp).Next; a.rflag = h->rflag.p;
  {
    const DenseTail &dt = (*h->anp).dt;
    a.dt.s = dt.s; a.dt.k = dt.k; a.dt.n_phases = dt.n_phases; a.dt.n_steps = dt.n_steps;
    a.dt.task = h->dt_task.p; a.dt.wave_task = h->dt_wave_task.p; a.dt.wave_step = h->dt_wave_step.p; a.dt.tail_bar = h->dt_tail_bar.p;
    a.dt_val = h->dt_val.p;
  }
  const Settings &s = h->st;
  a.sigma = s.sigma; a.alpha = s.alpha; a.eps_abs = s.eps_abs; a.eps_rel = s.eps_rel;
  a.eps_prim_inf = s.eps_prim_inf; a.eps_dual_inf = s.eps_dual_inf; a.rho_tolerance = s.adaptive_rho_tolerance;
  a.check_termination = (int)s.check_termination; a.rho_interval = (int)s.adaptive_rho_interval;
  a.max_iter = (int)s.max_iter; a.scaled_termination = (int)s.scaled_termination; a.scaling = s.scaling ? 1 : 0;
  a.adaptive_rho = (int)s.adaptive_rho; a.iter_begin = 0; a.iter_end = 0; a.info_at_end = 1;
  return a;
}

static FactorArgs make_factor_args(mi_osqp_batch *h, int force_all) {
  FactorArgs a{};
  const Analysis &an = (*h->anp);
  a.n = an.n; a.m = an.m; a.N = an.N; a.B = h->B; a.nnzP = an.Pp[an.n]; a.nnzK = an.nnzK();
  a.pa_len = an.Pp[an.n] + an.Ap[an.n]; a.n_levels = an.bf.n_levels; a.force_all = force_all;
  a.storage = an.bf.storage; a.fwd = h->fwd.view(an.fwd); a.bwd = h->bwd.view(an.bwd);
  a.blk = h->bf_blk.p; a.lvl = h->bf_lvl.p; a.utask = h->bf_utask.p; a.tri4 = h->bf_tri.p; a.dtask = h->bf_dtask.p; a.ubig = h->bf_ubig.p;
  a.ttask = h->bf_ttask.p; a.asm_dst = h->bf_asm_dst.p; a.asm_src = h->bf_asm_src.p;
  a.fwd_srcblk = h->fwd_srcblk.p; a.bwd_srcblk = h->bwd_srcblk.p;
  a.pa_val = h->pa_val.p; a.l = h->l.p; a.u = h->u.p; a.dscal = h->dscal.p;
  a.rho_vec = h->rho_vec.p; a.rho_inv = h->rho_inv.p; a.Lblk = h->Lblk.p; a.Dl = h->Dl.p; a.dinv_scratch = h->dinv_scratch.p;
  a.fwd_val = h->fwd_val.p; a.bwd_val = h->bwd_val.p; a.dinv = h->dinv.p; a.iscal = h->iscal.p; a.npos = h->npos.p; a.use_work = h->use_work.p;
  a.sigma = h->st.sigma; a.home_bt = h->BT; a.dt_k = an.dt.k;
// ... 282 lines not shown
  if (!tu.threads && !wide && BT <= 2 && !tu.global_xs && lds_bytes((int)(n + m), BT, 1024) <= lds_cap) {
    int dev = (int)device, cus = 256;
    if (dev < 0 && hipGetDevice(&dev) != hipSuccess) dev = 0;
    if (hipDeviceGetAttribute(&cus, hipDeviceAttributeMultiprocessorCount, dev) != hipSuccess || cus <= 0) cus = 256;
    (void)hipGetLastError();
    const int64_t tiles = (B + BT - 1) / BT;
    if (tiles <= cus || lds_bytes((int)(n + m), BT, 1024) > 80 * 1024) h->threads = 1024;
  }
  h->global_xs = wide || lds_bytes((int)(n + m), BT, h->threads) > lds_cap || tu.global_xs;
  int max_extra = -1;
  if (!h->global_xs) {
    const size_t cap_rows = (lds_cap - lds_bytes(0, BT, h->threads)) / (sizeof(double) * BT);
    max_extra = (int)(cap_rows - (size_t)(n + m));
  }
  h->mw_groups = 0; h->mw_threads = 0;
  if (h->global_xs && BT == 1 && B == 1 && h->threads <= 512) {
    const int64_t Nrows = n + m;
    h->mw_groups = tu.groups >= 0 ? tu.groups : (Nrows >= 250000 ? 256 : Nrows >= 60000 ? 128 : Nrows >= 30000 ? 64 : 32);
    h->mw_threads = tu.group_threads ? tu.group_threads : 128;
    if (h->mw_groups * (h->mw_threads / 64) > 2048) h->mw_groups = 2048 / (h->mw_threads / 64);
    int dev = (int)device, cus = 0;
    if ((dev >= 0 || hipGetDevice(&dev) == hipSuccess) && hipDeviceGetAttribute(&cus, hipDeviceAttributeMultiprocessorCount, dev) == hipSuccess && cus > 0) {
      DevGuard guard(dev);
      if (tu.assume_cus > 0) cus = std::min(cus, tu.assume_cus);
      const int cap = max_coresident_groups(h->mw_threads, lds_bytes(0, 1, h->threads), cus);
      if (cap > 0 && h->mw_groups > cap) h->mw_groups = cap;
      if (h->mw_groups == 1) h->mw_groups = 0;
    }
    (void)hipGetLastError();
  }
  BT_out = BT; max_extra_out = max_extra;
}

static int shape_and_analysis(mi_osqp_batch *h, int64_t B, int64_t n, int64_t m, const int64_t *Pp, const int64_t *Pi, const int64_t *Ap,
                              const int64_t *Ai, int64_t device, int &BT, int &max_extra, std::shared_ptr<const Analysis> &out) {
  derive_shape(h, B, n, m, device, BT, max_extra);
  int rc = cached_analysis(n, m, Pp, Pi, Ap, Ai, h->tune, h->threads / 64, BT, max_extra, h->global_xs ? 0 : 512, h->mw_groups * (h->mw_threads / 64), (int)((B + BT - 1) / BT), out);
  if (rc) return rc;
  const size_t lds_cap = 160 * 1024 - 1024;
  if (out->dt.k > 0 && (BT != 1 || h->threads != 1024) && !h->global_xs && !h->tune.tile && !h->tune.threads &&
      lds_bytes((int)(n + m), 1, 1024) + (size_t)2 * 512 * sizeof(double) <= lds_cap) {
    const int BT2 = 1, thr2 = 1024;
    const size_t cap_rows = (lds_cap - lds_bytes(0, BT2, thr2)) / (sizeof(double) * BT2);
    const int max_extra2 = (int)(cap_rows - (size_t)(n + m));
    std::shared_ptr<const Analysis> an2;
    rc = cached_analysis(n, m, Pp, Pi, Ap, Ai, h->tune, thr2 / 64, BT2, max_extra2, 512, 0, (int)B, an2);
    if (!rc && an2->dt.k > 0) { BT = BT2; h->threads = thr2; max_extra = max_extra2; out = an2; }
  }
  return MI_OSQP_OK;
}

static int batch_setup_impl(mi_osqp_batch *h, int64_t B, int64_t n, int64_t m, const int64_t *Pp, const int64_t *Pi,
                            const double *Pv, const double *q, const int64_t *Ap, const int64_t *Ai,
                            const double *Av, const double *l, const double *u, int64_t device) {
  double t0 = now_s();
  if (B <= 0 || !Pp || !Ap || (m > 0 && (!l || !u)) || (Pp[n] > 0 && !Pv) || (Ap[n] > 0 && !Av)) return MI_OSQP_ERR_INVALID_DATA;
  if (validate_settings(h->st)) return MI_OSQP_ERR_INVALID_SETTINGS;
  if (h->st.adaptive_rho && !h->st.adaptive_rho_interval) {
    h->rho_interval_auto = true;
    h->st.adaptive_rho_interval = h->st.check_termination ? 4 * h->st.check_termination : 100;
  }
  for (int64_t k = 0; k < B * m; k++) if (l[k] > u[k]) return MI_OSQP_ERR_INVALID_DATA;
  int BT = 1, max_extra = -1;
  const size_t lds_cap = 160 * 1024 - 1024;
  h->tune = tuning_from_env();
  const double ta0 = now_s();
  int rc = shape_and_analysis(h, B, n, m, Pp, Pi, Ap, Ai, device, BT, max_extra, h->anp);
  const double t_analysis = now_s() - ta0;
  if (rc) return rc;
  const Analysis &an = (*h->anp);
  h->B = (int)B;
  h->failed.assign((size_t)B, 0);
  int ndev = 0;
  if (hipGetDeviceCount(&ndev) != hipSuccess || ndev <= 0) { g_last_error = "no HIP device visible"; return MI_OSQP_ERR_DEVICE; }
  if (device >= ndev) { g_last_error = "no such HIP device"; return MI_OSQP_ERR_DEVICE; }
  if (device >= 0) h->device = (int)device; else HIPCHK(hipGetDevice(&h->device));
  DevGuard guard(h->device);
  hipDeviceProp_t prop;
  HIPCHK(hipGetDeviceProperties(&prop, h->device));
  h->n_cus = prop.multiProcessorCount > 0 ? prop.multiProcessorCount : 256;
  if (strncmp(prop.gcnArchName, "gfx950", 6) != 0) { g_last_error = std::string("device is not gfx950: ") + prop.gcnArchName; return MI_OSQP_ERR_DEVICE; }
  {
    streampool::Bundle sb;
    if (streampool::take(h->device, sb)) {
      h->stream = sb.stream; h->ev0 = sb.ev[0]; h->ev1 = sb.ev[1]; h->evf0 = sb.ev[2]; h->evf1 = sb.ev[3]; h->evf2 = sb.ev[4];
      h->pipe_r = sb.pipe_r; h->pipe_i = sb.pipe_i; h->pipe_x = sb.pipe_x;
      for (int k = 0; k < streampool::kPipeEvents; k++) h->pipe_ev[k] = sb.pipe_ev[k];
    }
    else {
      HIPCHK(hipStreamCreateWithFlags(&h->stream, hipStreamNonBlocking));
      HIPCHK(hipEventCreate(&h->ev0)); HIPCHK(hipEventCreate(&h->ev1));
      HIPCHK(hipEventCreate(&h->evf0)); HIPCHK(hipEventCreate(&h->evf1)); HIPCHK(hipEventCreate(&h->evf2));
    }
  }
  h->BT = BT; h->ntiles = (int)((B + BT - 1) / BT);
  h->lds = h->global_xs ? lds_bytes(0, BT, h->threads) : lds_bytes(an.Next + 2 * an.dt.k, BT, h->threads);
  if (h->lds > lds_cap) { g_last_error = "internal: LDS budget exceeded"; return MI_OSQP_ERR_ALLOC; }
  h->lds_iter = h->lds; h->rs_off = 0;
  {
    const size_t state = sizeof(double) * (size_t)BT * (2 * (size_t)n + 6 * (size_t)m + (size_t)an.N);
    if (!h->tune.stream_state && !h->global_xs && h->mw_groups <= 0 && h->threads == 1024 && h->lds + state <= lds_cap) {
      h->rs_off = (int)(h->lds / sizeof(double)); h->lds_iter = h->lds + state;
    }
  }
  h->lds_factor = 0; h->rf_off = 0; h->rf_steps = 0;
  if (h->rs_off && BT == 1 && an.dt.k > 0 && !h->tune.stream_factor) {
    const size_t part = (size_t)(h->threads / 64) * rf_lds_steps() * 64 * sizeof(double);
    if (h->lds_iter + part <= lds_cap) {
      h->rf_off = (int)(h->lds_iter / sizeof(double)); h->lds_factor = part;
      h->rf_steps = rf_head_steps(h->tune.rf_form == kIterDeepRing ? RF_FORM_DEEP_RING : RF_FORM_LONG_HEAD);
    }
  }
  size_t T = (size_t)h->ntiles * BT;
  if ((rc = h->fwd.upload(an.fwd)) || (rc = h->bwd.upload(an.bwd)) || (rc = h->chk.upload(an.chk))) return rc;
  { std::vector<uint32_t> pv(an.pinv.begin(), an.pinv.end()); if ((rc = h->pinv.upload(pv))) return rc; }
  { std::vector<uint32_t> xv(an.xloc.begin(), an.xloc.end()); if ((rc = h->xloc.upload(xv))) return rc; }
  {
    std::vector<int32_t> pr(an.Pi.begin(), an.Pi.begin() + an.Pp[n]), pc(an.Pp[n]), ar(an.Ai.begin(), an.Ai.begin() + an.Ap[n]), ac(an.Ap[n]);
    for (int j = 0; j < n; j++) { for (int k = an.Pp[j]; k < an.Pp[j + 1]; k++) pc[k] = j; for (int k = an.Ap[j]; k < an.Ap[j + 1]; k++) ac[k] = j; }
    if ((rc = h->rz_prow.upload(pr)) || (rc = h->rz_pcol.upload(pc)) || (rc = h->rz_arow.upload(ar)) || (rc = h->rz_acol.upload(ac))) return rc;
  }
  if ((rc = h->use_work.alloc(T)) || (rc = h->use_work.zero(h->stream))) return rc;
#define ALLOC(buf, len) if ((rc = h->buf.alloc((size_t)(len) * T)) || (rc = h->buf.zero(h->stream))) return rc
  ALLOC(fwd_val, (size_t)an.fwd.phys_steps() * 64); ALLOC(bwd_val, (size_t)an.bwd.phys_steps() * 64); ALLOC(chk_val, (size_t)an.chk.phys_steps() * 64); ALLOC(dinv, an.N);
  ALLOC(x, n); ALLOC(z, m); ALLOC(y, m); ALLOC(q, n); ALLOC(l, m); ALLOC(u, m); ALLOC(rho_vec, m); ALLOC(rho_inv, m);
  ALLOC(Dsc, n); ALLOC(Dsc_inv, n); ALLOC(Esc, m); ALLOC(Esc_inv, m); ALLOC(dx, n); ALLOC(dy, m);
  ALLOC(out1, 2 * n + m); ALLOC(out2, 2 * n + m); ALLOC(dscal, DS_COUNT);
  if (h->global_xs) { ALLOC(xs_global, an.xs_total); }
  if ((rc = h->mw_bar.alloc(4 * (size_t)std::max(h->n_cus, 1))) || (rc = h->mw_bar.zero(h->stream))) return rc;
  if (an.df && ((rc = h->rflag.upload(an.rflag)) || (rc = h->mw_scratch.alloc((size_t)8 * 256 * 16)) || (rc = h->mw_scratch.zero(h->stream)))) return rc;
  if (an.dt.k) {
    const DenseTail &dt = an.dt;
    ALLOC(dt_val, (size_t)dt.n_steps * 64);
    if ((rc = h->dt_task.upload(dt.task)) || (rc = h->dt_wave_task.upload(dt.wave_task)) || (rc = h->dt_wave_step.upload(dt.wave_step)) ||
        (rc = h->dt_tail_bar.upload(dt.tail_bar)) || (rc = h->dt_src.upload(dt.src)) ||
        (rc = h->dt_lt_pos.upload(dt.lt_pos)) || (rc = h->dt_ltcol_col.upload(dt.ltcol_col)) || (rc = h->dt_tile_tab.upload(dt.tile_tab)) ||
        (rc = h->dt_wave_tiles.upload(dt.wave_tiles)) || (rc = h->dt_asm_q64.upload(dt.asm_q64)) ||
        (rc = h->dt_src_tile.upload(dt.src_tile)) || (rc = h->dt_diag_tile.upload(dt.diag_tile)) || (rc = h->dt_task_step.upload(dt.task_step)) ||
        (rc = h->dt_Sd.alloc((size_t)dt.k * dt.k * (T + 4)))) return rc;
    const int nrt = dt.k / 16 - 4;
    h->dt_nh = nrt <= 14 ? std::max(nrt, 1) : (nrt + 1) / 2;
    h->dt_cs_doubles = (uint32_t)std::max(h->dt_nh * 1024, 64 * 65 + 63) / 64 * 64;
    h->dt_lds = std::max<size_t>((size_t)h->dt_cs_doubles + 4096, 2 * 64 * 65) * sizeof(double);
    h->dt_lds_asm = (dt.asm_lds_bytes() + 255) & ~(size_t)255;
    if (h->dt_lds > lds_cap || h->dt_lds_asm > lds_cap) { g_last_error = "internal: LDS budget of tail_kernel exceeded"; return MI_OSQP_ERR_ALLOC; }
  }
#undef ALLOC
  if ((rc = h->iscal.alloc((size_t)IS_COUNT * T)) || (rc = h->flag.alloc(4))) return rc;
  {
    const BlockFactor &bf = an.bf;
    if ((rc = h->bf_blk.upload(bf.blk)) || (rc = h->bf_lvl.upload(bf.lvl)) || (rc = h->bf_ubig.upload(bf.ubig)) || (rc = h->bf_utask.upload(bf.utask4)) ||
        (rc = h->bf_tri.upload(bf.tri4)) || (rc = h->bf_dtask.upload(bf.dtask4)) || (rc = h->bf_ttask.upload(bf.ttask4)) ||
        (rc = h->bf_asm_dst.upload(bf.asm_dst)) || (rc = h->bf_asm_src.upload(bf.asm_src)) ||
        (rc = h->fwd_srcblk.upload(an.fwd_srcblk)) || (rc = h->bwd_srcblk.upload(an.bwd_srcblk))) return rc;
    if ((rc = h->pa_val.alloc((size_t)(an.Pp[n] + an.Ap[n]) * T)) || (rc = h->pa_val.zero(h->stream)) ||
        (rc = h->Lblk.alloc((size_t)bf.storage * (T + 4))) || (rc = h->Dl.alloc((size_t)an.N * (T + 4))) || (rc = h->Dl.zero(h->stream)) ||
        (rc = h->dinv_scratch.alloc((size_t)an.N * (T + 4))) || (rc = h->npos.alloc(T))) return rc;
    HIPCHK(hostpool::alloc((void **)&h->h_npos, T * sizeof(int), &h->h_npos_cap));
  }
  if (!h->global_xs && an.Pp[n] + an.Ap[n] < 65536 && n + m < 65536 &&
      spmv_fused_lds_bytes((int)n, (int)m, an.Pp[n] + an.Ap[n], BT) <= 150 * 1024) {
    const int nnzP = an.Pp[n];
    std::vector<std::vector<uint32_t>> rows((size_t)2 * n + m);
    for (int c = 0; c < (int)n; c++)
      for (int k = an.Pp[c]; k < an.Pp[c + 1]; k++) {
        const int r = an.Pi[k];
        rows[r].push_back((uint32_t)k | ((uint32_t)c << 16));
        if (r != c) rows[c].push_back((uint32_t)k | ((uint32_t)r << 16));
      }
    for (int c = 0; c < (int)n; c++)
      for (int k = an.Ap[c]; k < an.Ap[c + 1]; k++) {
        const int r = an.Ai[k];
        rows[(size_t)n + c].push_back((uint32_t)(nnzP + k) | ((uint32_t)(n + r) << 16));
        rows[(size_t)2 * n + r].push_back((uint32_t)(nnzP + k) | ((uint32_t)c << 16));
      }
    std::vector<uint32_t> ptr{0u}, ent;
// ... 273 lines not shown
static int ensure_polish_buffers(mi_osqp_batch *h) {
  if (h->pol_stat.p) return MI_OSQP_OK;
  const Analysis &an = (*h->anp);
  const size_t T = (size_t)h->ntiles * h->BT;
  int rc;
  if ((rc = h->pol_fwd.alloc(h->fwd_val.n)) || (rc = h->pol_fwd.zero(h->stream)) || (rc = h->pol_bwd.alloc(h->bwd_val.n)) ||
      (rc = h->pol_bwd.zero(h->stream)) || (rc = h->pol_dinv.alloc(h->dinv.n)) || (rc = h->pol_dinv.zero(h->stream)) ||
      (rc = h->pol_sol.alloc(T * an.N)) || (rc = h->pol_act.alloc(std::max<size_t>(1, T * an.m))) || (rc = h->pol_act.zero(h->stream)) ||
      (rc = h->pol_stat.alloc(T)) || (rc = h->pol_stat.zero(h->stream))) return rc;
  if (an.dt.k && ((rc = h->pol_dt.alloc(h->dt_val.n)) || (rc = h->pol_dt.zero(h->stream)))) return rc;
  if (!h->evp0) HIPCHK(hipEventCreate(&h->evp0));
  if (!h->evp1) HIPCHK(hipEventCreate(&h->evp1));
  return MI_OSQP_OK;
}

static constexpr int kPolishInner = 4;

static int polish_impl(mi_osqp_batch *h, const KernelArgs &a) {
  const int BT = h->BT, ntl = h->ntiles;
  int rc;
  h->pol_count = h->pol_accepted = 0; h->pol_seconds = 0.0;
  h->pol_status.assign((size_t)h->B, 0);
  if ((rc = ensure_polish_buffers(h))) return rc;
  std::vector<int> work = koptimal_slots(h);
  PolishArgs pa{h->pol_stat.p, h->pol_act.p, h->pol_sol.p, (int)h->st.polish_refine_iter, kPolishInner, h->st.delta};
  HIPCHK(hipEventRecord(h->evp0, h->stream));
  HIPCHK(launch_polish_active(a, pa, BT, h->stream));
  const int n_pol = (int)work.size();
  if (n_pol) {
    if ((rc = device_refactor_slots(h, std::move(work), nullptr, &pa))) return rc;
    if ((rc = run_spinning(h, h->stream, [&]() -> int {
          HIPCHK(launch_polish(polish_stream_args(h, a), pa, BT, ntl, h->mw_groups > 0 ? h->mw_threads : h->threads, h->lds, h->n_cus, h->stream));
          HIPCHK(hipEventRecord(h->evp1, h->stream));
          return MI_OSQP_OK;
        }))) return rc;
  } else {
    HIPCHK(hipEventRecord(h->evp1, h->stream));
  }
  HIPCHK(hipMemcpyAsync(h->pol_status.data(), h->pol_stat.p, (size_t)h->B * sizeof(int), hipMemcpyDeviceToHost, h->stream));
  HIPCHK(hipStreamSynchronize(h->stream));
  float ms = 0.f;
  HIPCHK(hipEventElapsedTime(&ms, h->evp0, h->evp1));
  h->pol_seconds = ms * 1e-3;
  h->pol_count = n_pol;
  for (int v : h->pol_status) h->pol_accepted += v == 1;
  return MI_OSQP_OK;
}

static int adjoint_impl(mi_osqp_batch *h, const AdjointArgs &ga, int32_t *d_status, hipStream_t user_stream) {
  hipStream_t keep = h->stream;
  struct Restore { mi_osqp_batch *h; hipStream_t s; ~Restore() { h->stream = s; } } restore{h, keep};
  if (user_stream) h->stream = user_stream;
  const Analysis &an = (*h->anp);
  const int BT = h->BT, ntl = h->ntiles;
  int rc;
  if ((rc = ensure_polish_buffers(h))) return rc;
  if (!h->adj_stat.p && ((rc = h->adj_stat.alloc((size_t)ntl * BT)))) return rc;
  if ((rc = h->adj_stat.zero(h->stream))) return rc;
  std::vector<int> work;
  if (h->solved_once) {
    HIPCHK(hipMemcpyAsync(h->h_iscal, h->iscal.p, (size_t)ntl * IS_COUNT * BT * sizeof(int), hipMemcpyDeviceToHost, h->stream));
    HIPCHK(hipStreamSynchronize(h->stream));
    work = koptimal_slots(h);
  }
  if (!work.empty()) {
    const KernelArgs a = make_args(h);
    PolishArgs pa{h->adj_stat.p, h->pol_act.p, h->pol_sol.p, (int)h->st.polish_refine_iter};
    HIPCHK(launch_polish_active(a, pa, BT, h->stream));
    if ((rc = device_refactor_slots(h, std::move(work), nullptr, &pa))) return rc;
    if ((rc = run_spinning(h, h->stream, [&]() -> int {
          HIPCHK(launch_adjoint(polish_stream_args(h, a), pa, ga, BT, ntl, h->mw_groups > 0 ? h->mw_threads : h->threads, h->lds, h->n_cus, h->stream));
          return MI_OSQP_OK;
        }))) return rc;
  }
  HIPCHK(launch_adjoint_finish(h->adj_stat.p, ga, d_status, h->B, an.n, an.m, h->stream));
  HIPCHK(hipStreamSynchronize(h->stream));
  return MI_OSQP_OK;
}

struct PipeRegion {
  bool open = false;
  int iter = 0, n_chunks = 0, n_lanes = 1;
  bool tail = false;
  double host_s = 0.0;
  std::vector<int> work, wl, tiles;
  std::vector<int> lane_last;
};
constexpr int kDefaultLanes = 2;
constexpr bool kDefaultChunk0First = false;
static bool pipeline_applies(const mi_osqp_batch *h, int n_ref) {
  const int longer_than = h->tune.pipeline_min > 0 ? h->tune.pipeline_min : h->n_cus;
  return h->tune.refactor_pipeline && n_ref > longer_than && h->mw_groups <= 0 && !h->global_xs && !(*h->anp).wide && !(*h->anp).df;
}

struct RunAhead {
  bool open = false;
  bool used = false;
  int chk_threads = 0;
  std::vector<int> points;
  std::vector<int> group, rest, work;
  std::vector<int> ru0;
};
constexpr int kRunaheadQuarters = 2;
static bool runahead_applies(const mi_osqp_batch *h) {
  const int lanes = h->tune.refactor_lanes > 0 ? h->tune.refactor_lanes : kDefaultLanes;
  return h->tune.runahead && h->tune.refactor_pipeline && h->BT == 1 && lanes <= 2 && h->st.adaptive_rho && h->st.adaptive_rho_interval > 0 &&
         h->mw_groups <= 0 && !h->global_xs && !(*h->anp).wide && !(*h->anp).df;
}
static int ensure_runahead_buffers(mi_osqp_batch *h) {
  int rc;
  if (!h->ra_list.p && (rc = h->ra_list.alloc((size_t)5 * h->ntiles))) return rc;
  if (!h->ra_res.p && (rc = h->ra_res.alloc((size_t)2 * h->ntiles))) return rc;
  if (!h->h_res) HIPCHK(hostpool::alloc((void **)&h->h_res, (size_t)2 * h->ntiles * sizeof(double), &h->h_res_cap));
  if (!h->h_mark) HIPCHK(hostpool::alloc((void **)&h->h_mark, (size_t)h->ntiles * sizeof(int), &h->h_mark_cap));
  return 0;
}

static int pipelined_refactor_iterate(mi_osqp_batch *h, const KernelArgs &a, const std::vector<int> &work, const std::vector<int> &active, PipeRegion *pr,
                                      const RunAhead *ra = nullptr) {
  using streampool::kPipeChunks; using streampool::kPipeEvents; using streampool::kPipeLanes;
  const double t_begin = now_s();
  const int BT = h->BT, nq = (int)work.size();
  int rc;
  if (!h->pipe_r) HIPCHK(hipStreamCreateWithFlags(&h->pipe_r, hipStreamNonBlocking));
  if (!h->pipe_i) HIPCHK(hipStreamCreateWithFlags(&h->pipe_i, hipStreamNonBlocking));
  for (int k = 0; k < kPipeEvents; k++) if (!h->pipe_ev[k]) HIPCHK(hipEventCreate(&h->pipe_ev[k]));
  hipEvent_t ev_fork = h->pipe_ev[0], ev_i0 = h->pipe_ev[1], ev_join = h->pipe_ev[2];
  auto ev_chunk = [&](int c, int k) { return h->pipe_ev[3 + 3 * (c - 1) + k]; };
  auto ev_lane = [&](int l) { return h->pipe_ev[3 + 3 * kPipeChunks + l]; };
  int n_even = h->tune.pipeline_chunks > 0 ? h->tune.pipeline_chunks : (nq + h->n_cus - 1) / h->n_cus;
  int chunk_qps = (nq + n_even - 1) / n_even;
  if (h->tune.pipeline_chunks <= 0 && h->tune.pipeline_chunk_qps > 0) chunk_qps = h->tune.pipeline_chunk_qps;
  const RefactorChunks ch = refactor_chunks(work, active, BT, chunk_qps, kPipeChunks);
  const int kbt = nq <= h->n_cus ? 1 : BT;
  const int lanes_asked = h->tune.refactor_lanes > 0 ? h->tune.refactor_lanes : kDefaultLanes;
  const RefactorLanes rl = refactor_lanes(ch, work, BT, kbt, std::min(lanes_asked, kPipeLanes), h->tune.lanes_chunk0 < 0 ? kDefaultChunk0First : h->tune.lanes_chunk0 != 0,
                                          h->ntiles * BT + 4);
  const int L = rl.n_lanes;
  if (L > 2 && !h->pipe_x) HIPCHK(hipStreamCreateWithFlags(&h->pipe_x, hipStreamNonBlocking));
  if (ra && (L > 2 || BT != 1)) { g_last_error = "run-ahead beside three chunk lanes / tiles of several QPs"; return MI_OSQP_ERR_INVALID_SETTINGS; }
  std::vector<int> &wl = pr->wl;
  std::vector<int> wl_begin(1, 0);
  wl.clear();
  for (int c = 1; c < ch.n_chunks; c++) {
    wl.insert(wl.end(), work.begin() + ch.work_begin[c], work.begin() + ch.work_begin[c + 1]);
    wl.resize((wl.size() + kbt - 1) / kbt * kbt, -1);
    wl_begin.push_back((int)wl.size());
  }
  pr->tiles = ch.tiles; pr->work = work;
  if (h->work.n < wl.size() && (rc = h->work.alloc((size_t)h->ntiles * BT + 4 + (size_t)BT * kPipeChunks))) return rc;
  if (h->tile_list.n < ch.tiles.size() && (rc = h->tile_list.alloc((size_t)h->ntiles))) return rc;
  HIPCHK(hipMemcpyAsync(h->work.p, wl.data(), wl.size() * sizeof(int), hipMemcpyHostToDevice, h->stream));
  HIPCHK(hipMemcpyAsync(h->tile_list.p, pr->tiles.data(), pr->tiles.size() * sizeof(int), hipMemcpyHostToDevice, h->stream));
  const int ntl = h->ntiles, G = ra ? (int)ra->group.size() : 0, gw = ra ? (int)ra->work.size() : 0;
  int *d_rest = h->ra_list.p, *d_group = d_rest + ntl, *d_gwork = d_rest + 2 * (size_t)ntl, *d_dwork = d_rest + 3 * (size_t)ntl, *d_mark = d_rest + 4 * (size_t)ntl;
  if (ra) {
    if (!h->ra_list.p || G <= 0 || G + (int)ra->rest.size() != ntl || gw > G || nq + G > ntl + 4) { g_last_error = "run-ahead: inconsistent lists"; return MI_OSQP_ERR_INVALID_SETTINGS; }
    if (!ra->rest.empty()) HIPCHK(hipMemcpyAsync(d_rest, ra->rest.data(), ra->rest.size() * sizeof(int), hipMemcpyHostToDevice, h->stream));
    HIPCHK(hipMemcpyAsync(d_group, ra->group.data(), (size_t)G * sizeof(int), hipMemcpyHostToDevice, h->stream));
    if (gw) HIPCHK(hipMemcpyAsync(d_gwork, ra->work.data(), (size_t)gw * sizeof(int), hipMemcpyHostToDevice, h->stream));
    HIPCHK(hipMemsetAsync(d_mark, 0, (size_t)ntl * sizeof(int), h->stream));
  }
  pr->host_s = now_s() - t_begin;
  HIPCHK(hipEventRecord(ev_fork, h->stream));
  FactorArgs fa = make_factor_args(h, 0);
  const bool tail = (*h->anp).dt.k != 0;
  auto enqueue_refactor = [&](int c, int base, hipStream_t st) -> int {
    const int *wc = h->work.p + wl_begin[c - 1];
    const int slots = wl_begin[c] - wl_begin[c - 1];
    fa.work = wc; fa.wg_base = base / kbt;
    HIPCHK(hipEventRecord(ev_chunk(c, 0), st));
    HIPCHK(launch_factor(fa, kbt, slots / kbt, h->tune.factor_threads, st));
    HIPCHK(hipEventRecord(ev_chunk(c, 1), st));
    if (tail) {
      TailArgs da = make_tail_args(h, kbt, wc);
      da.wg_base = base;
      HIPCHK(launch_tail(da, slots, h->dt_lds_asm, h->dt_lds, st));
    }
    HIPCHK(hipEventRecord(ev_chunk(c, 2), st));
    return 0;
  };
  KernelArgs ai = a;
  auto enqueue_iterate = [&](int c, hipStream_t st) -> int {
    const int nt = ch.tile_begin[c + 1] - ch.tile_begin[c];
    if (!nt) return 0;
    ai.tiles = h->tile_list.p + ch.tile_begin[c];
    ai.rf_form = iterate_form(nt, h->rf_off != 0, h->tune);
    h->rf_launches[ai.rf_form]++;
    HIPCHK(launch_iterate(ai, BT, nt, h->threads, h->lds_iter + h->lds_factor, st));
    return 0;
  };
  hipStream_t sx = h->stream;
  KernelArgs ac = a;
  ac.tiles = d_group; ac.res = nullptr; ac.info_at_end = 1;
  FactorArgs fg = make_factor_args(h, 0);
  fg.wg_base = nq;
  auto chain_refactor = [&](const int *list, int n, int iter) -> int {
    if (n <= 0) return 0;
    fg.work = list;
    HIPCHK(launch_factor(fg, 1, n, h->tune.factor_threads, sx));
    if (tail) {
      TailArgs da = make_tail_args(h, 1, list);
      da.wg_base = nq;
      HIPCHK(launch_tail(da, n, h->dt_lds_asm, h->dt_lds, sx));
    }
    HIPCHK(launch_fail_flagged(a, list, n, BT, iter, sx, d_mark));
    return 0;
  };
  auto chain_segment = [&](size_t k) -> int {
    ac.iter_begin = k ? ra->points[k - 1] : a.iter_begin; ac.iter_end = ra->points[k];
    ac.rf_form = iterate_form(G, h->rf_off != 0, h->tune);
    h->rf_launches[ac.rf_form]++;
    HIPCHK(launch_iterate(ac, BT, G, h->threads, h->lds_iter + h->lds_factor, sx));
    HIPCHK(launch_check(ac, BT, G, ra->chk_threads, h->lds, sx));
    const int e = ra->points[k];
    if (k + 1 < ra->points.size() && e % (int)h->st.adaptive_rho_interval == 0) {
      HIPCHK(launch_worklist_of(h->iscal.p, d_group, d_dwork, G, BT, sx));
      return chain_refactor(d_dwork, G, e);
    }
    return 0;
  };
  if (ra) {
    if ((rc = chain_refactor(d_gwork, gw, a.iter_begin)) || (rc = chain_segment(0))) return rc;
  }
  pr->lane_last.assign(L, 0);
  if (L == 1) {
    HIPCHK(hipStreamWaitEvent(h->pipe_r, ev_fork, 0));
    HIPCHK(hipStreamWaitEvent(h->pipe_i, ev_fork, 0));
    for (int c = 1; c < ch.n_chunks; c++) if ((rc = enqueue_refactor(c, 0, h->pipe_r))) return rc;
    pr->lane_last[0] = ch.n_chunks - 1;
    HIPCHK(hipEventRecord(ev_i0, h->pipe_i));
    for (int c = 0; c < ch.n_chunks; c++) {
      if (c) HIPCHK(hipStreamWaitEvent(h->pipe_i, ev_chunk(c, 2), 0));
      if ((rc = enqueue_iterate(c, h->pipe_i))) return rc;
    }
    HIPCHK(hipEventRecord(ev_lane(0), h->pipe_i));
  } else {
    hipStream_t lane[kPipeLanes] = {h->pipe_r, h->pipe_i, h->pipe_x};
    for (int l = 0; l < L; l++) HIPCHK(hipStreamWaitEvent(lane[l], ev_fork, 0));
    const bool chunk0_first = rl.order[rl.lane_of[0]].front() == 0;
    if (chunk0_first && (rc = enqueue_iterate(0, lane[rl.lane_of[0]]))) return rc;
    size_t w = 0;
    for (int c = 1; c < ch.n_chunks; c++) {
      const int l = rl.lane_of[c];
      if ((rc = enqueue_refactor(c, rl.scratch_begin[c], lane[l]))) return rc;
      pr->lane_last[l] = c;
      for (; w < rl.wait_chunk.size() && rl.wait_chunk[w] == c; w++) HIPCHK(hipStreamWaitEvent(lane[l], ev_chunk(rl.wait_for[w], 2), 0));
      if ((rc = enqueue_iterate(c, lane[l]))) return rc;
    }
    if (!chunk0_first && (rc = enqueue_iterate(0, lane[rl.lane_of[0]]))) return rc;
    for (int l = 0; l < L; l++) HIPCHK(hipEventRecord(ev_lane(l), lane[l]));
  }
  if (ra) for (size_t k = 1; k < ra->points.size(); k++) if ((rc = chain_segment(k))) return rc;
  for (int l = 0; l < L; l++) HIPCHK(hipStreamWaitEvent(h->stream, ev_lane(l), 0));
  HIPCHK(hipEventRecord(ev_join, h->stream));
  HIPCHK(launch_fail_flagged(a, h->work.p, (int)wl.size(), BT, a.iter_begin, h->stream));
  pr->open = true; pr->iter = a.iter_begin; pr->n_chunks = ch.n_chunks; pr->n_lanes = L; pr->tail = tail;
  h->refactor_lanes = std::max<int64_t>(h->refactor_lanes, L);
  return 0;
}

static int pipelined_region_finish(mi_osqp_batch *h, PipeRegion *pr) {
  using streampool::kPipeChunks;
  if (!pr->open) return 0;
  pr->open = false;
  const int BT = h->BT, nq = (int)pr->work.size();
  hipEvent_t ev_fork = h->pipe_ev[0], ev_i0 = h->pipe_ev[1], ev_join = h->pipe_ev[2];
  auto ev_chunk = [&](int c, int k) { return h->pipe_ev[3 + 3 * (c - 1) + k]; };
  float f_ms = 0.f, d_ms = 0.f, r_ms = 0.f, i_ms = 0.f, w_ms = 0.f;
  for (int c = 1; c < pr->n_chunks; c++) {
    float f = 0.f, d = 0.f;
    HIPCHK(hipEventElapsedTime(&f, ev_chunk(c, 0), ev_chunk(c, 1))); HIPCHK(hipEventElapsedTime(&d, ev_chunk(c, 1), ev_chunk(c, 2)));
    f_ms += f; d_ms += pr->tail ? d : 0.f;
  }
  for (int c : pr->lane_last) {
    float r = 0.f;
    if (c) HIPCHK(hipEventElapsedTime(&r, ev_fork, ev_chunk(c, 2)));
    r_ms = std::max(r_ms, r);
  }
  HIPCHK(hipEventElapsedTime(&w_ms, ev_fork, ev_join));
  if (pr->n_lanes == 1) HIPCHK(hipEventElapsedTime(&i_ms, ev_i0, h->pipe_ev[3 + 3 * kPipeChunks])); else i_ms = w_ms;
  const double wall = pr->host_s + 1e-3 * std::max(w_ms, r_ms), ref_s = pr->host_s + 1e-3 * r_ms;
  h->last_refactor_s += ref_s; h->last_device_s += wall - ref_s;
  h->kernel_ms_sum += i_ms; h->kernel_launches++; h->last_launches++;
  h->factor_ms_sum += f_ms; h->dense_ms_sum += d_ms; h->refactor_launches++; h->refactor_qps += nq;
  if (nq >= h->peak_qps) { h->peak_qps = nq; h->peak_factor_ms = f_ms; h->peak_tail_ms = d_ms; }
  h->pipelined_refactors++;
  for (int s : pr->work)
    if (s >= 0 && s < h->B && h->h_iscal[(size_t)(s / BT) * IS_COUNT * BT + IS_STATUS * BT + s % BT] == -7) h->failed[s] = 1;
  return 0;
}

static int solve_impl(mi_osqp_batch *h, double *d_x_out, hipStream_t user_stream) {
  hipStream_t keep = h->stream;
  struct Restore { mi_osqp_batch *h; hipStream_t s; ~Restore() { h->stream = s; } } restore{h, keep};
  if (user_stream) h->stream = user_stream;
  int rc;
  if ((rc = reset_solve_state(h, !h->st.warm_start))) return rc;
  KernelArgs a = make_args(h);
  if (d_x_out) a.x_out = d_x_out;
  h->last_total_iters = h->last_launches = h->last_refactors = 0;
  h->last_device_s = h->last_refactor_s = 0.0;
  const int BT = h->BT, ntl = h->ntiles, nslots = ntl * BT;
  const Settings &S = h->st;
  int iterating = ntl;
  {
    std::vector<int> bad;
    for (int q = 0; q < h->B; q++) if (h->failed[q]) bad.push_back(q);
    if ((rc = fail_slots(h, a, bad, 0))) return rc;
  }
  auto segment_end = [&](int iter) {
    int seg_end = (int)S.max_iter;
    if (S.check_termination > 0) seg_end = std::min<int64_t>(seg_end, (iter / S.check_termination + 1) * S.check_termination);
    if (S.adaptive_rho && S.adaptive_rho_interval > 0)
      seg_end = std::min<int64_t>(seg_end, (iter / S.adaptive_rho_interval + 1) * S.adaptive_rho_interval);
    return seg_end;
  };
  const int ra_min = h->tune.runahead_min > 0 ? h->tune.runahead_min : h->n_cus;
  if (runahead_applies(h) && ntl > 1 && ntl >= ra_min) {
    if ((rc = ensure_runahead_buffers(h))) return rc;
    a.res = h->ra_res.p;
  }
  auto is_rho_point = [&](int iter) { return S.adaptive_rho && S.adaptive_rho_interval > 0 && iter % S.adaptive_rho_interval == 0; };
  auto loop = [&]() -> int {
    int iter = 0;
    bool iterated = false;
    PipeRegion region;
    RunAhead ra;
    std::vector<char> held;
    std::vector<int> left;
    const int *d_tiles = nullptr;
    int n_launch = ntl, res_iter = -1;
    bool leftovers_phase = false;
    auto check_threads = [&]() {
      int chk_threads = h->mw_groups > 0 ? h->mw_threads : h->threads;
      if (h->mw_groups <= 0 && h->threads == 1024 && ntl > 2 * h->n_cus) chk_threads = 512;
      return chk_threads;
    };
    auto device_turn = [&](int seg_end) -> int {
      a.iter_begin = iter; a.iter_end = seg_end; a.info_at_end = 1; a.tiles = d_tiles;
      {
        std::unique_lock<std::mutex> spin_lock(spin_mutex(h->device), std::defer_lock);
        if (h->mw_groups > 0) spin_lock.lock();
        if (!iterated) {
          HIPCHK(hipEventRecord(h->ev0, h->stream));
          if (h->mw_groups > 0) HIPCHK(hipMemsetAsync(h->mw_bar.p, 0, 4 * sizeof(uint32_t), h->stream));
          a.rf_form = iterate_form(iterating, h->rf_off != 0, h->tune);
          h->rf_launches[a.rf_form]++;
          HIPCHK(launch_iterate(a, BT, n_launch, h->mw_groups > 0 ? h->mw_threads : h->threads, h->lds_iter + h->lds_factor, h->stream));
          HIPCHK(hipEventRecord(h->ev1, h->stream));
        }
        HIPCHK(launch_check(a, BT, n_launch, check_threads(), h->lds, h->stream));
        HIPCHK(hipMemcpyAsync(h->h_iscal, h->iscal.p, (size_t)ntl * IS_COUNT * BT * sizeof(int), hipMemcpyDeviceToHost, h->stream));
        if (a.res && !ra.used && is_rho_point(seg_end) && seg_end < S.max_iter) {
          HIPCHK(hipMemcpyAsync(h->h_res, h->ra_res.p, (size_t)2 * ntl * sizeof(double), hipMemcpyDeviceToHost, h->stream));
          res_iter = seg_end;
        }
        if (ra.open) HIPCHK(hipMemcpyAsync(h->h_mark, h->ra_list.p + 4 * (size_t)ntl, (size_t)ntl * sizeof(int), hipMemcpyDeviceToHost, h->stream));
        HIPCHK(hipStreamSynchronize(h->stream));
      }
      if ((rc = mw_barrier_ok(h))) {
        const std::string why = g_last_error;
        (void)restore_snapshot(h);
        g_last_error = why + " (the handle is back in the state of its last setup / update, cold-started)";
        return rc;
      }
      if (!iterated) {
        float ms = 0.f;
        HIPCHK(hipEventElapsedTime(&ms, h->ev0, h->ev1));
        h->last_device_s += ms * 1e-3; h->kernel_ms_sum += ms; h->kernel_launches++; h->last_launches++;
      } else if ((rc = pipelined_region_finish(h, &region))) return rc;
      iterated = false;
      if (ra.open) {
        ra.open = false;
        int64_t inner = 0, n_left = 0;
        for (size_t i = 0; i < ra.group.size(); i++) {
          const int t = ra.group[i];
          const int *f = h->h_iscal + (size_t)t * IS_COUNT;
          const bool flagged = f[IS_NEED_REFACTOR] == 1;
          inner += f[IS_RHO_UPDATES] - ra.ru0[i] - (flagged ? 1 : 0);
          if (h->h_mark[t]) h->failed[(size_t)t] = 1;
          n_left += !f[IS_DONE];
          if (!f[IS_DONE] || flagged) left.push_back(t);
        }
        std::sort(left.begin(), left.end());
        h->last_refactors += inner; h->refactor_qps += (int64_t)ra.work.size() + inner;
        h->ra_left += n_left;
        if (left.empty()) { d_tiles = nullptr; n_launch = ntl; }
        else { held.assign((size_t)nslots, 0); for (int t : left) held[(size_t)t] = 1; }
      }
      return 0;
    };
    auto host_turn = [&](bool *go_on) -> int {
      *go_on = false;
      std::vector<int> active, work;
      for (int s = 0; s < h->B; s++) {
        if (!held.empty() && held[(size_t)s]) continue;
        const int *t = h->h_iscal + (size_t)(s / BT) * IS_COUNT * BT;
        if (!t[IS_DONE * BT + s % BT]) active.push_back(s);
        if (t[IS_NEED_REFACTOR * BT + s % BT]) work.push_back(s);
      }
      if (ra.used && !leftovers_phase && ra.points.size() && iter == segment_end(ra.points[0])) h->ra_missed += (int64_t)active.size();
      const int n_ref = (int)work.size();
      if (active.empty() && !n_ref) return 0;
      if (n_ref) {
        double tr = now_s();
        std::vector<int> bad;
        int rc2;
        if (!active.empty() && pipeline_applies(h, n_ref)) {
          KernelArgs nx = a;
          nx.iter_begin = iter; nx.iter_end = segment_end(iter); nx.info_at_end = 1;
          std::vector<int> work_m, active_m;
          if (a.res && !ra.used && res_iter == iter) {
            std::vector<double> pri(active.size()), dua(active.size());
            for (size_t i = 0; i < active.size(); i++) { pri[i] = h->h_res[2 * (size_t)active[i]]; dua[i] = h->h_res[2 * (size_t)active[i] + 1]; }
            const int size = h->tune.runahead_tiles > 0 ? h->tune.runahead_tiles : std::max(1, h->n_cus * kRunaheadQuarters / 4);
            std::vector<int> group = runahead_group(active, pri, dua, size, ra_min);
            if (!group.empty() && group.size() < active.size()) {
              std::vector<char> in((size_t)nslots, 0);
              for (int t : group) in[(size_t)t] = 1;
              for (int s : work) (in[(size_t)s] ? ra.work : work_m).push_back(s);
              for (int s : active) if (!in[(size_t)s]) active_m.push_back(s);
              if (pipeline_applies(h, (int)work_m.size())) {
                for (int t = 0; t < ntl; t++) if (!in[(size_t)t]) ra.rest.push_back(t);
                for (int t : group) ra.ru0.push_back(h->h_iscal[(size_t)t * IS_COUNT + IS_RHO_UPDATES]);
                const int interval = (int)S.adaptive_rho_interval;
                const int end = (int)std::min<int64_t>(S.max_iter, (int64_t)(iter / interval + 2) * interval);
                for (int it = iter; it < end && (h->tune.runahead_end <= 0 || (int)ra.points.size() < h->tune.runahead_end);) ra.points.push_back(it = segment_end(it));
                ra.group = std::move(group); ra.chk_threads = check_threads();
                ra.used = ra.open = true;
              } else ra.work.clear();
            }
          }
          if (ra.open) {
            if ((rc2 = pipelined_refactor_iterate(h, nx, work_m, active_m, &region, &ra))) return rc2;
            d_tiles = h->ra_list.p; n_launch = (int)ra.rest.size();
            h->ra_regions++; h->ra_tiles += (int64_t)ra.group.size();
          } else if ((rc2 = pipelined_refactor_iterate(h, nx, work, active, &region))) return rc2;
          iterated = true;
          tr = now_s();
        } else if ((rc2 = device_refactor_slots(h, std::move(work), &bad))) return rc2;
        if ((rc2 = fail_slots(h, a, bad, iter))) return rc2;
        h->host_rho_stale = true;
        h->last_refactors += n_ref;
        h->last_refactor_s += now_s() - tr;
        if (!bad.empty()) {
          std::vector<char> isbad(nslots, 0);
          for (int q : bad) isbad[q] = 1;
          active.erase(std::remove_if(active.begin(), active.end(), [&](int q) { return isbad[q] != 0; }), active.end());
        }
      }
      if (active.empty()) return 0;
      iterating = 0;
      for (size_t i = 0; i < active.size(); i++) iterating += !i || active[i] / BT != active[i - 1] / BT;
      *go_on = true;
      return 0;
    };
    while (true) {
      const int seg_end = segment_end(iter);
      if ((rc = device_turn(seg_end))) return rc;
      iter = seg_end;
      bool go_on = false;
      if ((rc = host_turn(&go_on))) return rc;
      if (go_on) continue;
      if (leftovers_phase || left.empty()) break;
      leftovers_phase = true;
      held.assign((size_t)nslots, 1);
      for (int t : left) held[(size_t)t] = 0;
      HIPCHK(hipMemcpyAsync(h->ra_list.p, left.data(), left.size() * sizeof(int), hipMemcpyHostToDevice, h->stream));
      d_tiles = h->ra_list.p; n_launch = (int)left.size();
      a.tiles = d_tiles;
      iter = ra.points.back();
      if ((rc = host_turn(&go_on))) return rc;
      if (!go_on) break;
    }
    return MI_OSQP_OK;
  };
  rc = loop();
  a.tiles = nullptr; a.res = nullptr;
  if (rc) {
    if (h->pipe_r) (void)hipStreamSynchronize(h->pipe_r);
    if (h->pipe_i) (void)hipStreamSynchronize(h->pipe_i);
    if (h->pipe_x) (void)hipStreamSynchronize(h->pipe_x);
    (void)hipStreamSynchronize(h->stream);
    return rc;
  }
  HIPCHK(hipMemcpyAsync(h->h_iscal, h->iscal.p, (size_t)nslots * IS_COUNT * sizeof(int), hipMemcpyDeviceToHost, h->stream));
  HIPCHK(hipStreamSynchronize(h->stream));
  for (int qi = 0; qi < h->B; qi++)
    h->last_total_iters += h->h_iscal[(size_t)(qi / BT) * IS_COUNT * BT + IS_ITER * BT + qi % BT];
  h->solved_once = true;
  if (h->st.polish && (rc = polish_impl(h, a))) return rc;
  if (!h->st.polish) { h->pol_status.clear(); h->pol_count = h->pol_accepted = 0; }
  return MI_OSQP_OK;
}


extern "C" {

void mi_osqp_default_settings(mi_osqp_settings *s) {
  if (!s) return;
  s->rho = 0.1; s->sigma = 1e-6; s->scaling = 10; s->adaptive_rho = 1; s->adaptive_rho_interval = 0;
  s->adaptive_rho_tolerance = 5.0; s->max_iter = 4000; s->eps_abs = 1e-3; s->eps_rel = 1e-3;
  s->eps_prim_inf = 1e-4; s->eps_dual_inf = 1e-4; s->alpha = 1.6; s->scaled_termination = 0;
  s->check_termination = 25; s->warm_start = 1; s->verbose = 0;
  s->polish = 0; s->polish_refine_iter = 3; s->delta = 1e-6;
}

const char *mi_osqp_exit_code_name(int64_t c) {
  static const char *names[] = {"kOptimal", "kPrimalInfeasible", "kDualInfeasible", "kOptimalInaccurate",
                                "kPrimalInfeasibleInaccurate", "kDualInfeasibleInaccurate", "kMaxIterations",
                                "kInterrupted", "kTimeLimitReached", "kNonConvex", "kUnknown"};
  return (c >= 0 && c <= 10) ? names[c] : "kUnknown";
}
const char *mi_osqp_error_name(int64_t e) {
  static const char *names[] = {"ok", "invalid data", "invalid settings", "sparsity pattern changed",
                                "non-convex problem / KKT inertia", "device error", "null argument", "allocation / size"};
  return (e >= 0 && e <= 7) ? names[e] : "unknown";
}
const char *mi_osqp_version(void) { return "mi-osqp 0.2 (gfx950)"; }
const char *mi_osqp_last_error(void) { return g_last_error.c_str(); }

static int64_t exit_code_of(int status) {
  switch (status) {
    case 1: return MI_OSQP_EXIT_OPTIMAL;
    case 2: return MI_OSQP_EXIT_OPTIMAL_INACCURATE;
    case -3: return MI_OSQP_EXIT_PRIMAL_INFEASIBLE;
    case 3: return MI_OSQP_EXIT_PRIMAL_INFEASIBLE_INACCURATE;
    case -4: return MI_OSQP_EXIT_DUAL_INFEASIBLE;
    case 4: return MI_OSQP_EXIT_DUAL_INFEASIBLE_INACCURATE;
    case -2: return MI_OSQP_EXIT_MAX_ITERATIONS;
    case -5: return MI_OSQP_EXIT_INTERRUPTED;
    case -6: return MI_OSQP_EXIT_TIME_LIMIT_REACHED;
    case -7: return MI_OSQP_EXIT_NON_CONVEX;
    default: return MI_OSQP_EXIT_UNKNOWN;
  }
}

int mi_osqp_batch_setup(mi_osqp_batch **out, int64_t B, int64_t n, int64_t m, const int64_t *Pp, const int64_t *Pi,
                        const double *Pv, const double *q, const int64_t *Ap, const int64_t *Ai, const double *Av,
                        const double *l, const double *u, const mi_osqp_settings *settings, int64_t device) {
  CallTimer timer_("batch_setup");
  if (!out) return MI_OSQP_ERR_NULL;
  *out = nullptr;
  if (n <= 0 || m < 0) return MI_OSQP_ERR_INVALID_DATA;
  mi_osqp_batch *h = new (std::nothrow) mi_osqp_batch();
  if (!h) return MI_OSQP_ERR_ALLOC;
  h->st = to_settings(settings);
  int rc = batch_setup_impl(h, B, n, m, Pp, Pi, Pv, q, Ap, Ai, Av, l, u, device);
  if (rc) { delete h; return rc; }
  *out = h;
  return MI_OSQP_OK;
}

int mi_osqp_prefetch_analysis(int64_t B, int64_t n, int64_t m, const int64_t *Pp, const int64_t *Pi, const int64_t *Ap, const int64_t *Ai, int64_t device) {
  CallTimer timer_("prefetch_analysis");
  if (B <= 0 || n <= 0 || m < 0 || !Pp || !Ap || (Pp[n] > 0 && !Pi) || (Ap[n] > 0 && !Ai)) return MI_OSQP_ERR_INVALID_DATA;
  mi_osqp_batch tmp;
  tmp.tune = tuning_from_env();
  int BT = 1, max_extra = -1;
  std::shared_ptr<const Analysis> an;
  return shape_and_analysis(&tmp, B, n, m, Pp, Pi, Ap, Ai, device, BT, max_extra, an);
}

void mi_osqp_batch_free(mi_osqp_batch *h) { delete h; }
void mi_osqp_release_device_cache(void) { devpool::release_all(); hostpool::release_all(); streampool::release_all(); }
// ... 108 lines not shown
  if (!h->pol_act.p) { memset(act, 0, cnt); return MI_OSQP_OK; }
  DevGuard guard(h->device);
  if (h->cont.on) HIPCHK(hipStreamSynchronize(h->stream));
  if (cnt) HIPCHK(hipMemcpy(act, h->pol_act.p, cnt, hipMemcpyDeviceToHost));
  return MI_OSQP_OK;
}

static AdjointArgs adjoint_args(mi_osqp_batch *h, const double *d_dx, const double *d_dy, double *d_dq, double *d_dP, double *d_dA,
                                double *d_dl, double *d_du) {
  const Analysis &an = (*h->anp);
  AdjointArgs ga{};
  ga.gx = d_dx; ga.gy = d_dy; ga.dq = d_dq; ga.dP = d_dP; ga.dA = d_dA; ga.dl = d_dl; ga.du = d_du;
  ga.prow = h->rz_prow.p; ga.pcol = h->rz_pcol.p; ga.arow = h->rz_arow.p; ga.acol = h->rz_acol.p;
  ga.nnzP = (int)an.Pp[an.n]; ga.nnzA = (int)an.Ap[an.n];
  return ga;
}
int mi_osqp_batch_adjoint_device(mi_osqp_batch *h, const double *d_dx, const double *d_dy, double *d_dq, double *d_dP, double *d_dA,
                                 double *d_dl, double *d_du, int32_t *d_status, void *stream) {
  CallTimer timer_("batch_adjoint_device");
  if (!h) return MI_OSQP_ERR_NULL;
  if (!d_dx) { g_last_error = "adjoint: dx is null (dL/dx is required; only dy may be null)"; return MI_OSQP_ERR_NULL; }
  for (const double *o : {(const double *)d_dq, (const double *)d_dP, (const double *)d_dA, (const double *)d_dl, (const double *)d_du})
    if (o && (o == d_dx || o == d_dy)) { g_last_error = "adjoint: an output aliases dx or dy"; return MI_OSQP_ERR_INVALID_DATA; }
  DevGuard guard(h->device);
  { const int rc_ = cont_leave(h); if (rc_) return rc_; }
  return adjoint_impl(h, adjoint_args(h, d_dx, d_dy, d_dq, d_dP, d_dA, d_dl, d_du), d_status, (hipStream_t)stream);
}
int mi_osqp_batch_adjoint(mi_osqp_batch *h, const double *dx, const double *dy, double *dq, double *dP, double *dA, double *dl,
                          double *du, int32_t *status) {
  CallTimer timer_("batch_adjoint");
  if (!h) return MI_OSQP_ERR_NULL;
  if (!dx) { g_last_error = "adjoint: dx is null (dL/dx is required; only dy may be null)"; return MI_OSQP_ERR_NULL; }
  DevGuard guard(h->device);
  { const int rc_ = cont_leave(h); if (rc_) return rc_; }
  const Analysis &an = (*h->anp);
  const size_t B = (size_t)h->B, n = (size_t)an.n, m = (size_t)an.m, nnzP = (size_t)an.Pp[an.n], nnzA = (size_t)an.Ap[an.n];
  const size_t len[7] = {B * n, dy ? B * m : 0, dq ? B * n : 0, dP ? B * nnzP : 0, dA ? B * nnzA : 0, dl ? B * m : 0, du ? B * m : 0};
  size_t off[8] = {0};
  for (int k = 0; k < 7; k++) off[k + 1] = off[k] + len[k];
  DevBuf<double> buf;
  DevBuf<int> stat;
  int rc;
  if ((rc = buf.alloc(off[7])) || (rc = stat.alloc(B))) return rc;
  auto at = [&](int k) -> double * { return len[k] ? buf.p + off[k] : nullptr; };
  HIPCHK(hipMemcpy(at(0), dx, len[0] * sizeof(double), hipMemcpyHostToDevice));
  if (len[1]) HIPCHK(hipMemcpy(at(1), dy, len[1] * sizeof(double), hipMemcpyHostToDevice));
  if ((rc = adjoint_impl(h, adjoint_args(h, at(0), at(1), at(2), at(3), at(4), at(5), at(6)), stat.p, nullptr))) return rc;
  double *out[7] = {nullptr, nullptr, dq, dP, dA, dl, du};
  for (int k = 2; k < 7; k++) if (len[k]) HIPCHK(hipMemcpy(out[k], at(k), len[k] * sizeof(double), hipMemcpyDeviceToHost));
  if (status) HIPCHK(hipMemcpy(status, stat.p, B * sizeof(int32_t), hipMemcpyDeviceToHost));
  return MI_OSQP_OK;
}

int mi_osqp_batch_get_scaling(mi_osqp_batch *h, double *D, double *E, double *c) {
  if (!h || !D || !E || !c) return MI_OSQP_ERR_NULL;
  DevGuard guard(h->device);
  { const int rc_ = cont_leave(h); if (rc_) return rc_; }
  const int n = (*h->anp).n, m = (*h->anp).m, B = h->B, BT = h->BT;
  int rc;
  if ((rc = ensure_stage(h, (size_t)B * std::max({n, m, 1}) + 1, 0))) return rc;
  auto down = [&](const double *src, int len, double *dst) -> int {
    if (!len) return 0;
    HIPCHK(launch_deinterleave(src, h->stage.p, B, len, BT, h->stream));
    HIPCHK(hipMemcpyAsync(dst, h->stage.p, (size_t)B * len * sizeof(double), hipMemcpyDeviceToHost, h->stream));
    HIPCHK(hipStreamSynchronize(h->stream));
    return 0;
  };
  if ((rc = down(h->Dsc.p, n, D)) || (rc = down(h->Esc.p, m, E))) return rc;
  const size_t dcnt = (size_t)h->ntiles * DS_COUNT * BT;
  HIPCHK(hipMemcpy(h->h_dscal, h->dscal.p, dcnt * sizeof(double), hipMemcpyDeviceToHost));
  for (int q = 0; q < B; q++) c[q] = h->h_dscal[(size_t)(q / BT) * DS_COUNT * BT + DS_C * BT + q % BT];
  return MI_OSQP_OK;
}

int mi_osqp_batch_get_stats(mi_osqp_batch *h, mi_osqp_stats *st) {
  if (!h || !st) return MI_OSQP_ERR_NULL;
  *st = h->stats;
  st->pipelined_refactors = h->pipelined_refactors;
  st->refactor_lanes = h->refactor_lanes;
  st->iterate_launches_deep_ring = h->rf_launches[RF_FORM_DEEP_RING];
  st->iterate_launches_long_head = h->rf_launches[RF_FORM_LONG_HEAD];
  st->runahead_regions = h->ra_regions; st->runahead_tiles = h->ra_tiles;
  st->runahead_left = h->ra_left; st->runahead_missed = h->ra_missed;
  return MI_OSQP_OK;
}

int mi_osqp_batch_get_ordering(mi_osqp_batch *h, int64_t *kkt_perm) {
  if (!h || !kkt_perm) return MI_OSQP_ERR_NULL;
  const Analysis &an = (*h->anp);
  for (int k = 0; k < an.N; k++) kkt_perm[k] = an.perm[(size_t)k];
  return MI_OSQP_OK;
}

int mi_osqp_batch_last_solve_stats(mi_osqp_batch *h, int64_t *total_iters, int64_t *kernel_launches, double *device_seconds,
                                   double *refactor_seconds, int64_t *refactor_count, double *compact_seconds) {
  if (!h) return MI_OSQP_ERR_NULL;
  if (compact_seconds) *compact_seconds = 0.0;
  if (total_iters) *total_iters = h->last_total_iters;
  if (kernel_launches) *kernel_launches = h->last_launches;
  if (device_seconds) *device_seconds = h->last_device_s;
  if (refactor_seconds) *refactor_seconds = h->last_refactor_s;
  if (refactor_count) *refactor_count = h->last_refactors;
  return MI_OSQP_OK;
}

int mi_osqp_batch_kernel_time(mi_osqp_batch *h, double *avg_ms, int64_t *launches) {
  if (!h) return MI_OSQP_ERR_NULL;
  if (avg_ms) *avg_ms = h->kernel_launches ? h->kernel_ms_sum / (double)h->kernel_launches : 0.0;
  if (launches) *launches = h->kernel_launches;
  h->kernel_ms_sum = 0.0; h->kernel_launches = 0;
  return MI_OSQP_OK;
}

int mi_osqp_batch_refactor_time(mi_osqp_batch *h, double *factor_ms, double *dense_ms, int64_t *launches, int64_t *qps) {
  if (!h) return MI_OSQP_ERR_NULL;
  if (factor_ms) *factor_ms = h->factor_ms_sum;
  if (dense_ms) *dense_ms = h->dense_ms_sum;
  if (launches) *launches = h->refactor_launches;
  if (qps) *qps = h->refactor_qps;
  h->factor_ms_sum = h->dense_ms_sum = 0.0; h->refactor_launches = h->refactor_qps = 0;
  h->peak_qps = 0; h->peak_factor_ms = h->peak_tail_ms = 0.0;
  return MI_OSQP_OK;
}

int mi_osqp_batch_refactor_peak(mi_osqp_batch *h, int64_t *qps, double *factor_ms, double *tail_ms) {
  if (!h) return MI_OSQP_ERR_NULL;
  if (qps) *qps = h->peak_qps;
  if (factor_ms) *factor_ms = h->peak_factor_ms;
  if (tail_ms) *tail_ms = h->peak_tail_ms;
  return MI_OSQP_OK;
}

int mi_osqp_batch_reset(mi_osqp_batch *h) {
  CallTimer timer_("batch_reset");
  if (!h) return MI_OSQP_ERR_NULL;
  DevGuard guard(h->device);
  { const int rc_ = cont_leave(h); if (rc_) return rc_; }
  return restore_snapshot(h);
}
}
static int restore_snapshot(mi_osqp_batch *h) {
  h->clear_rho_updates = true;
  auto cp = [&](DevBuf<double> &dst, DevBuf<double> &src) -> int {
    if (src.n) HIPCHK(hipMemcpyAsync(dst.p, src.p, src.n * sizeof(double), hipMemcpyDeviceToDevice, h->stream));
    return 0;
  };
  int rc;
  const size_t nflags = (size_t)h->ntiles * h->BT;
  HIPCHK(hipMemsetD32Async((hipDeviceptr_t)h->use_work.p, 0, nflags, h->stream));
  if ((rc = cp(h->dinv, h->dinv0)) || (rc = cp(h->rho_vec, h->rho_vec0)) || (rc = cp(h->rho_inv, h->rho_inv0)) || (rc = cp(h->dscal, h->dscal0))) return rc;
  if ((rc = reset_solve_state(h, true))) return rc;
  HIPCHK(hipStreamSynchronize(h->stream));
  h->host_rho_stale = true;
  return MI_OSQP_OK;
}
extern "C" {

int mi_osqp_batch_warm_start_x(mi_osqp_batch *h, const double *x) {
  CallTimer timer_("batch_warm_start_x");
  if (!h || !x) return MI_OSQP_ERR_NULL;
  DevGuard guard(h->device);
  { const int rc_ = cont_leave(h); if (rc_) return rc_; }
  h->st.warm_start = 1;
  size_t cnt = (size_t)h->B * (*h->anp).n;
  int rc;
  if ((rc = ensure_stage(h, cnt, 0)) || (rc = ensure_pin(h, cnt))) return rc;
// ... 1515 lines not shown
}

int mi_gomp_relinearise_some(mi_gomp_scene *sc, int64_t n_ids, const int64_t *ids, const double *x, int32_t *ok_out) {
  CallTimer timer_("gomp_relinearise_some");
  if (!sc || (n_ids > 0 && (!ids || !x || !ok_out))) return MI_OSQP_ERR_NULL;
  if (!n_ids) return MI_OSQP_OK;
  mi_osqp_batch *h = sc->h;
  DevGuard guard(h->device);
  int rc;
  if ((rc = cont_enter(h)) || (rc = cont_check_ids(h, n_ids, ids, true))) return rc;
  if ((rc = gomp_launch(sc, n_ids, ids, x, 2, ok_out))) return rc;
  std::vector<int64_t> bad;
  for (int64_t j = 0; j < n_ids; j++) if (!ok_out[j]) bad.push_back(ids[j]);
  if (bad.empty()) return MI_OSQP_OK;
  return cont_new_data(h, (int64_t)bad.size(), bad.data(), nullptr, nullptr, nullptr, false, sc->A.p, sc->l.p, sc->u.p);
}

}

extern "C" {


int mi_osqp_setup(mi_osqp_solver **out, int64_t n, int64_t m, const int64_t *Pp, const int64_t *Pi, const double *Pv,
                  const double *q, const int64_t *Ap, const int64_t *Ai, const double *Av, const double *l,
                  const double *u, const mi_osqp_settings *settings) {
  if (!out) return MI_OSQP_ERR_NULL;
  *out = nullptr;
  mi_osqp_batch *b = nullptr;
  int rc = mi_osqp_batch_setup(&b, 1, n, m, Pp, Pi, Pv, q, Ap, Ai, Av, l, u, settings, -1);
  if (rc) return rc;
  mi_osqp_solver *s = new (std::nothrow) mi_osqp_solver();
  if (!s) { delete b; return MI_OSQP_ERR_ALLOC; }
  s->b = b; *out = s;
  return MI_OSQP_OK;
}
void mi_osqp_free(mi_osqp_solver *h) { if (h) { delete h->b; delete h; } }
int mi_osqp_update_A_bounds(mi_osqp_solver *h, const int64_t *Ap, const int64_t *Ai, const double *Av, const double *l, const double *u) {
  return h ? mi_osqp_batch_update_A_bounds(h->b, Ap, Ai, Av, l, u) : MI_OSQP_ERR_NULL;
}
int mi_osqp_update_A(mi_osqp_solver *h, const int64_t *Ap, const int64_t *Ai, const double *Av) {
  return h ? mi_osqp_batch_update_A(h->b, Ap, Ai, Av) : MI_OSQP_ERR_NULL;
}
int mi_osqp_update_bounds(mi_osqp_solver *h, const double *l, const double *u) {
  return h ? mi_osqp_batch_update_bounds(h->b, l, u) : MI_OSQP_ERR_NULL;
}
int mi_osqp_warm_start_x(mi_osqp_solver *h, const double *x) { return h ? mi_osqp_batch_warm_start_x(h->b, x) : MI_OSQP_ERR_NULL; }
int mi_osqp_update_q(mi_osqp_solver *h, const double *q) { return h ? mi_osqp_batch_update_q(h->b, q) : MI_OSQP_ERR_NULL; }
int mi_osqp_update_P(mi_osqp_solver *h, const int64_t *Pp, const int64_t *Pi, const double *Pv) {
  return h ? mi_osqp_batch_update_P(h->b, Pp, Pi, Pv) : MI_OSQP_ERR_NULL;
}
int mi_osqp_update_P_A(mi_osqp_solver *h, const int64_t *Pp, const int64_t *Pi, const double *Pv, const int64_t *Ap, const int64_t *Ai,
                       const double *Av) {
  return h ? mi_osqp_batch_update_P_A(h->b, Pp, Pi, Pv, Ap, Ai, Av) : MI_OSQP_ERR_NULL;
}
int mi_osqp_warm_start_y(mi_osqp_solver *h, const double *y) { return h ? mi_osqp_batch_warm_start_y(h->b, y) : MI_OSQP_ERR_NULL; }
int mi_osqp_solve(mi_osqp_solver *h, mi_osqp_info *info) {
  if (!h) return MI_OSQP_ERR_NULL;
  int rc = mi_osqp_batch_solve(h->b);
  if (rc) return rc;
  if (info) return mi_osqp_batch_get_info(h->b, info);
  return MI_OSQP_OK;
}
int mi_osqp_get_primal(mi_osqp_solver *h, double *x) { return h ? mi_osqp_batch_get_primal(h->b, x) : MI_OSQP_ERR_NULL; }
int mi_osqp_get_dual(mi_osqp_solver *h, double *y) { return h ? mi_osqp_batch_get_dual(h->b, y) : MI_OSQP_ERR_NULL; }
int mi_osqp_get_prim_inf_cert(mi_osqp_solver *h, double *dy_out) { return h ? mi_osqp_batch_get_prim_inf_cert(h->b, dy_out) : MI_OSQP_ERR_NULL; }
int mi_osqp_get_dual_inf_cert(mi_osqp_solver *h, double *dx_out) { return h ? mi_osqp_batch_get_dual_inf_cert(h->b, dx_out) : MI_OSQP_ERR_NULL; }
int mi_osqp_adjoint(mi_osqp_solver *h, const double *dx, const double *dy, double *dq, double *dP, double *dA, double *dl, double *du,
                    int32_t *status) {
  return h ? mi_osqp_batch_adjoint(h->b, dx, dy, dq, dP, dA, dl, du, status) : MI_OSQP_ERR_NULL;
}
int mi_osqp_debug_refactor_chunks(int64_t n_flagged, const int64_t *flagged, int64_t n_active, const int64_t *active, int64_t tile,
                                  int64_t chunk_qps, int64_t max_chunks, int64_t *n_chunks, int64_t *work_begin, int64_t *tiles,
                                  int64_t *tile_begin) {
  if (!n_chunks || !work_begin || !tiles || !tile_begin || (n_flagged > 0 && !flagged) || (n_active > 0 && !active)) return MI_OSQP_ERR_NULL;
  if (n_flagged < 0 || n_active < 0 || tile < 1 || chunk_qps < 1 || max_chunks < 1) return MI_OSQP_ERR_INVALID_DATA;
  const std::vector<int> f(flagged, flagged + n_flagged), a(active, active + n_active);
  const RefactorChunks ch = refactor_chunks(f, a, (int)tile, (int)chunk_qps, (int)max_chunks);
  *n_chunks = ch.n_chunks;
  std::copy(ch.work_begin.begin(), ch.work_begin.end(), work_begin);
  std::copy(ch.tiles.begin(), ch.tiles.end(), tiles);
  std::copy(ch.tile_begin.begin(), ch.tile_begin.end(), tile_begin);
  return MI_OSQP_OK;
}
int mi_osqp_debug_refactor_lanes(int64_t n_flagged, const int64_t *flagged, int64_t n_active, const int64_t *active, int64_t tile,
                                 int64_t chunk_qps, int64_t max_chunks, int64_t kbt, int64_t lanes, int64_t chunk0_first,
                                 int64_t scratch_slots, int64_t *n_lanes, int64_t *lane_of, int64_t *order, int64_t *order_begin,
                                 int64_t *scratch_begin, int64_t *n_waits, int64_t *wait_chunk, int64_t *wait_for) {
  if (!n_lanes || !lane_of || !order || !order_begin || !scratch_begin || !n_waits || !wait_chunk || !wait_for ||
      (n_flagged > 0 && !flagged) || (n_active > 0 && !active)) return MI_OSQP_ERR_NULL;
  if (n_flagged < 0 || n_active < 0 || tile < 1 || chunk_qps < 1 || max_chunks < 1 || kbt < 1 || lanes < 1 || lanes > 3 || scratch_slots < 0)
    return MI_OSQP_ERR_INVALID_DATA;
  const std::vector<int> f(flagged, flagged + n_flagged), a(active, active + n_active);
  const RefactorChunks ch = refactor_chunks(f, a, (int)tile, (int)chunk_qps, (int)max_chunks);
  const RefactorLanes rl = refactor_lanes(ch, f, (int)tile, (int)kbt, (int)lanes, chunk0_first != 0, (int)std::min<int64_t>(scratch_slots, INT32_MAX));
  *n_lanes = rl.n_lanes;
  std::copy(rl.lane_of.begin(), rl.lane_of.end(), lane_of);
  order_begin[0] = 0;
  for (int l = 0; l < rl.n_lanes; l++) {
    std::copy(rl.order[l].begin(), rl.order[l].end(), order + order_begin[l]);
    order_begin[l + 1] = order_begin[l] + (int64_t)rl.order[l].size();
  }
  std::copy(rl.scratch_begin.begin(), rl.scratch_begin.begin() + ch.n_chunks, scratch_begin);
  *n_waits = (int64_t)rl.wait_chunk.size();
  std::copy(rl.wait_chunk.begin(), rl.wait_chunk.end(), wait_chunk);
  std::copy(rl.wait_for.begin(), rl.wait_for.end(), wait_for);
  return MI_OSQP_OK;
}
int mi_osqp_debug_runahead_group(int64_t n_active, const int64_t *tiles, const double *pri_res, const double *dua_res, int64_t size,
                                 int64_t min_active, int64_t *n_group, int64_t *group) {
  if (!n_group || !group || (n_active > 0 && (!tiles || !pri_res || !dua_res))) return MI_OSQP_ERR_NULL;
  if (n_active < 0 || n_active > INT32_MAX || size < 0 || size > INT32_MAX || min_active < 0 || min_active > INT32_MAX) return MI_OSQP_ERR_INVALID_DATA;
  std::vector<int> t((size_t)n_active);
  for (int64_t i = 0; i < n_active; i++) {
    if (tiles[i] < 0 || tiles[i] > INT32_MAX || pri_res[i] < 0.0 || dua_res[i] < 0.0) return MI_OSQP_ERR_INVALID_DATA;
    t[(size_t)i] = (int)tiles[i];
  }
  {
    std::vector<int> sorted = t;
    std::sort(sorted.begin(), sorted.end());
    if (std::adjacent_find(sorted.begin(), sorted.end()) != sorted.end()) return MI_OSQP_ERR_INVALID_DATA;
  }
  const std::vector<int> g = runahead_group(t, std::vector<double>(pri_res, pri_res + n_active), std::vector<double>(dua_res, dua_res + n_active),
                                            (int)size, (int)min_active);
  *n_group = (int64_t)g.size();
  std::copy(g.begin(), g.end(), group);
  return MI_OSQP_OK;
}
int mi_osqp_debug_iterate_form(int64_t tiles, int64_t has_head, int64_t forced_form, int64_t long_min, int64_t *form) {
  if (!form) return MI_OSQP_ERR_NULL;
  if (tiles < 0 || tiles > INT32_MAX || forced_form < 0 || forced_form > 2 || long_min < -1 || long_min > INT32_MAX)
    return MI_OSQP_ERR_INVALID_DATA;
  Tuning t;
  t.rf_form = (int)forced_form; t.rf_long_min = (int)long_min;
  *form = iterate_form((int)tiles, has_head != 0, t);
  return MI_OSQP_OK;
}
int mi_osqp_get_stats(mi_osqp_solver *h, mi_osqp_stats *st) { return h ? mi_osqp_batch_get_stats(h->b, st) : MI_OSQP_ERR_NULL; }
int mi_osqp_get_settings(mi_osqp_solver *h, mi_osqp_settings *out) { return h ? mi_osqp_batch_get_settings(h->b, out) : MI_OSQP_ERR_NULL; }
int mi_osqp_update_settings(mi_osqp_solver *h, const mi_osqp_settings *s) { return h ? mi_osqp_batch_update_settings(h->b, s) : MI_OSQP_ERR_NULL; }


}

struct ShardWorker {
  std::thread th;
  std::mutex mu;
  std::condition_variable cv;
  std::function<int()> job;
  bool has_job = false, busy = false, quit = false;
  int rc = 0;
  std::string err;
  void start() {
    th = std::thread([this] {
      std::unique_lock<std::mutex> lk(mu);
      for (;;) {
        cv.wait(lk, [this] { return has_job || quit; });
        if (quit) return;
        std::function<int()> f = std::move(job);
        has_job = false;
        lk.unlock();
        const int r = f();
        const std::string e = r ? g_last_error : std::string();
        lk.lock();
        rc = r; err = e; busy = false;
        cv.notify_all();
      }
// ... 281 lines not shown
```

Measured before the change: 43020.

## Size refactor region chunks by run-ahead width and add optional stream priorities

Chunk sizing for the pipelined refactor region now accounts for the run-ahead group width and the CU count: with run-ahead active it targets about twice as many chunks as rounds, capped at the pipe chunk limit. It also adds two opt-in options. One gives the lane or chain streams different priorities, running the run-ahead chain on a separate high-priority stream. The other runs the convergence and fail checks per lane instead of once after the join. By default only the chunk-sizing change takes effect, which alters how finely refactorisation overlaps with iteration and may add launch overhead.

```diff
diff --git a/include/mi_osqp.h b/include/mi_osqp.h
--- a/include/mi_osqp.h
+++ b/include/mi_osqp.h
@@ -84,6 +84,7 @@
   int64_t refactor_lanes;
   int64_t iterate_launches_deep_ring, iterate_launches_long_head;
   int64_t runahead_regions, runahead_tiles, runahead_left, runahead_missed;
+  int64_t region_priority, region_lane_checks, region_chunks;
 } mi_osqp_stats;
 
 typedef struct mi_osqp_solver mi_osqp_solver;
@@ -290,6 +291,8 @@
                                   int64_t chunk_qps, int64_t max_chunks, int64_t *n_chunks, int64_t *work_begin, int64_t *tiles,
                                   int64_t *tile_begin);
 
+int mi_osqp_debug_region_chunks(int64_t nq, int64_t gw, int64_t n_cus, int64_t *chunk_qps, int64_t *n_chunks);
+
 int mi_osqp_debug_refactor_lanes(int64_t n_flagged, const int64_t *flagged, int64_t n_active, const int64_t *active, int64_t tile,
                                  int64_t chunk_qps, int64_t max_chunks, int64_t kbt, int64_t lanes, int64_t chunk0_first,
                                  int64_t scratch_slots, int64_t *n_lanes, int64_t *lane_of, int64_t *order, int64_t *order_begin,
diff --git a/osqp-solver_amd/__init__.py b/osqp-solver_amd/__init__.py
--- a/osqp-solver_amd/__init__.py
+++ b/osqp-solver_amd/__init__.py
@@ -52,7 +52,8 @@
                 ("refactor_lanes", C.c_int64),
                 ("iterate_launches_deep_ring", C.c_int64), ("iterate_launches_long_head", C.c_int64),
                 ("runahead_regions", C.c_int64), ("runahead_tiles", C.c_int64), ("runahead_left", C.c_int64),
-                ("runahead_missed", C.c_int64)]
+                ("runahead_missed", C.c_int64),
+                ("region_priority", C.c_int64), ("region_lane_checks", C.c_int64), ("region_chunks", C.c_int64)]
 
     def as_dict(self):
         return {k: getattr(self, k) for k, _ in self._fields_}
@@ -193,6 +194,7 @@
         L.mi_osqp_debug_refactor_chunks.argtypes = [C.c_int64, ip, C.c_int64, ip, C.c_int64, C.c_int64, C.c_int64, ip, ip, ip, ip]
         L.mi_osqp_debug_refactor_lanes.argtypes = [C.c_int64, ip, C.c_int64, ip] + [C.c_int64] * 7 + [ip] * 8
         L.mi_osqp_debug_runahead_group.argtypes = [C.c_int64, ip, dp, dp, C.c_int64, C.c_int64, ip, ip]
+        L.mi_osqp_debug_region_chunks.argtypes = [C.c_int64] * 3 + [ip] * 2
         L.mi_osqp_debug_iterate_form.argtypes = [C.c_int64] * 4 + [ip]
         L.mi_osqp_prefetch_analysis.argtypes = [C.c_int64, C.c_int64, C.c_int64, ip, ip, ip, ip, C.c_int64]
         L.mi_osqp_debug_host_block_factor.argtypes = [C.c_int64, C.c_int64, ip, ip, dp, ip, ip, dp, dp, dp,
@@ -857,6 +859,12 @@
                 waits=list(zip(wc[:nw.value].tolist(), wf[:nw.value].tolist())))
 
 
+def debug_region_chunks(nq, gw, n_cus):
+    q, k = C.c_int64(), C.c_int64()
+    _chk(lib().mi_osqp_debug_region_chunks(nq, gw, n_cus, C.byref(q), C.byref(k)), "debug_region_chunks")
+    return int(q.value), int(k.value)
+
+
 def debug_runahead_group(tiles, pri_res, dua_res, size, min_active):
     t, p, d = _i64(tiles), _f64(pri_res), _f64(dua_res)
     if not (len(t) == len(p) == len(d)):
diff --git a/osqp-solver_amd/csrc/host_core.cpp b/osqp-solver_amd/csrc/host_core.cpp
--- a/osqp-solver_amd/csrc/host_core.cpp
+++ b/osqp-solver_amd/csrc/host_core.cpp
@@ -950,6 +950,8 @@
   if (const char *e = getenv("MI_OSQP_REFACTOR_CHUNK_QPS")) t.pipeline_chunk_qps = std::max(0, atoi(e));
   if (const char *e = getenv("MI_OSQP_REFACTOR_LANES")) t.refactor_lanes = std::max(1, std::min(3, atoi(e)));
   if (const char *e = getenv("MI_OSQP_REFACTOR_CHUNK0")) t.lanes_chunk0 = atoi(e) != 0;
+  if (const char *e = getenv("MI_OSQP_REGION_PRIORITY")) t.region_priority = std::max(0, std::min(2, atoi(e)));
+  if (const char *e = getenv("MI_OSQP_LANE_CHECKS")) t.lane_checks = atoi(e) != 0;
   if (const char *e = getenv("MI_OSQP_RUNAHEAD")) t.runahead = atoi(e) != 0;
   if (const char *e = getenv("MI_OSQP_RUNAHEAD_TILES")) t.runahead_tiles = std::max(0, atoi(e));
   if (const char *e = getenv("MI_OSQP_RUNAHEAD_MIN")) t.runahead_min = std::max(0, atoi(e));
@@ -990,6 +992,14 @@
   for (const auto &p : tc) { rc.tiles.push_back(p.second); rc.tile_begin[(size_t)p.first + 1]++; }
   for (int c = 0; c < rc.n_chunks; c++) rc.tile_begin[(size_t)c + 1] += rc.tile_begin[c];
   return rc;
+}
+
+int region_chunk_qps(int nq, int gw, int n_cus, int max_chunks) {
+  nq = std::max(0, nq); gw = std::max(0, gw); n_cus = std::max(1, n_cus);
+  const int64_t rounds = ((int64_t)nq + gw + n_cus - 1) / n_cus;
+  const int64_t want = gw > 0 ? 2 * rounds - 1 : rounds;
+  const int n_even = (int)std::max<int64_t>(1, std::min<int64_t>(want, std::min(std::max(1, max_chunks), std::max(1, nq))));
+  return (int)std::max<int64_t>(1, ((int64_t)nq + n_even - 1) / n_even);
 }
 
 RefactorLanes refactor_lanes(const RefactorChunks &ch, const std::vector<int> &flagged, int bt, int kbt, int lanes, bool chunk0_first, int scratch_slots) {
diff --git a/osqp-solver_amd/csrc/host_core.hpp b/osqp-solver_amd/csrc/host_core.hpp
--- a/osqp-solver_amd/csrc/host_core.hpp
+++ b/osqp-solver_amd/csrc/host_core.hpp
@@ -36,6 +36,8 @@
   }
 };
 constexpr bool kRunaheadDefault = true;
+constexpr int kRegionPriorityDefault = 0;
+constexpr bool kLaneChecksDefault = false;
 struct Tuning {
   int tile = 0;
   int threads = 0;
@@ -56,6 +58,8 @@
   int pipeline_chunk_qps = 0;
   int refactor_lanes = 0;
   int lanes_chunk0 = -1;
+  int region_priority = kRegionPriorityDefault;
+  bool lane_checks = kLaneChecksDefault;
   bool runahead = kRunaheadDefault;
   int runahead_tiles = 0;
   int runahead_min = 0;
@@ -77,6 +81,8 @@
   std::vector<int> tile_begin;
 };
 RefactorChunks refactor_chunks(const std::vector<int> &flagged, const std::vector<int> &active, int bt, int chunk_qps, int max_chunks);
+
+int region_chunk_qps(int nq, int gw, int n_cus, int max_chunks);
 
 struct RefactorLanes {
   int n_lanes = 1;
diff --git a/osqp-solver_amd/csrc/solver.hip b/osqp-solver_amd/csrc/solver.hip
--- a/osqp-solver_amd/csrc/solver.hip
+++ b/osqp-solver_amd/csrc/solver.hip
@@ -170,12 +170,12 @@
 namespace streampool {
 constexpr int kPipeChunks = 8;
 constexpr int kPipeLanes = 3;
-constexpr int kPipeEvents = 3 + 3 * kPipeChunks + kPipeLanes;
-struct Bundle { int dev; hipStream_t stream; hipEvent_t ev[5]; hipStream_t pipe_r, pipe_i, pipe_x; hipEvent_t pipe_ev[kPipeEvents]; };
+constexpr int kPipeEvents = 3 + 3 * kPipeChunks + kPipeLanes + 1;
+struct Bundle { int dev; hipStream_t stream; hipEvent_t ev[5]; hipStream_t pipe_r, pipe_i, pipe_x; hipEvent_t pipe_ev[kPipeEvents]; int lane_prio; hipStream_t pipe_c; };
 static void destroy(const Bundle &b) {
   for (hipEvent_t e : b.ev) if (e) (void)hipEventDestroy(e);
   for (hipEvent_t e : b.pipe_ev) if (e) (void)hipEventDestroy(e);
-  for (hipStream_t st : {b.stream, b.pipe_r, b.pipe_i, b.pipe_x}) if (st) (void)hipStreamDestroy(st);
+  for (hipStream_t st : {b.stream, b.pipe_r, b.pipe_i, b.pipe_x, b.pipe_c}) if (st) (void)hipStreamDestroy(st);
 }
 static std::mutex mu;
 static std::vector<Bundle> idle;
@@ -305,6 +305,10 @@
   hipEvent_t ev0 = nullptr, ev1 = nullptr, evf0 = nullptr, evf1 = nullptr, evf2 = nullptr;
   hipStream_t pipe_r = nullptr, pipe_i = nullptr, pipe_x = nullptr;
   hipEvent_t pipe_ev[streampool::kPipeEvents] = {};
+  int prio_form = 0, lane_prio = 0, chain_prio = 0;
+  bool prio_inert = false;
+  hipStream_t pipe_c = nullptr;
+  int64_t region_priority = 0, region_lane_checks = 0, region_chunks = 0;
   DevBuf<int> tile_list;
   int64_t pipelined_refactors = 0;
   int64_t refactor_lanes = 0;
@@ -374,7 +378,8 @@
     if (pipe_r) (void)hipStreamSynchronize(pipe_r);
     if (pipe_i) (void)hipStreamSynchronize(pipe_i);
     if (pipe_x) (void)hipStreamSynchronize(pipe_x);
-    streampool::Bundle sb{device, stream, {ev0, ev1, evf0, evf1, evf2}, pipe_r, pipe_i, pipe_x, {}};
+    if (pipe_c) (void)hipStreamSynchronize(pipe_c);
+    streampool::Bundle sb{device, stream, {ev0, ev1, evf0, evf1, evf2}, pipe_r, pipe_i, pipe_x, {}, lane_prio, pipe_c};
     for (int k = 0; k < streampool::kPipeEvents; k++) sb.pipe_ev[k] = pipe_ev[k];
     if (stream && ev0 && ev1 && evf0 && evf1 && evf2) streampool::give(sb);
     else streampool::destroy(sb);
@@ -823,9 +828,10 @@
   if (strncmp(prop.gcnArchName, "gfx950", 6) != 0) { g_last_error = std::string("device is not gfx950: ") + prop.gcnArchName; return MI_OSQP_ERR_DEVICE; }
   {
     streampool::Bundle sb;
-    if (streampool::take(h->device, sb)) {
+    const bool pooled = streampool::take(h->device, sb);
+    if (pooled) {
       h->stream = sb.stream; h->ev0 = sb.ev[0]; h->ev1 = sb.ev[1]; h->evf0 = sb.ev[2]; h->evf1 = sb.ev[3]; h->evf2 = sb.ev[4];
-      h->pipe_r = sb.pipe_r; h->pipe_i = sb.pipe_i; h->pipe_x = sb.pipe_x;
+      h->pipe_r = sb.pipe_r; h->pipe_i = sb.pipe_i; h->pipe_x = sb.pipe_x; h->pipe_c = sb.pipe_c;
       for (int k = 0; k < streampool::kPipeEvents; k++) h->pipe_ev[k] = sb.pipe_ev[k];
     }
     else {
@@ -833,6 +839,15 @@
       HIPCHK(hipEventCreate(&h->ev0)); HIPCHK(hipEventCreate(&h->ev1));
       HIPCHK(hipEventCreate(&h->evf0)); HIPCHK(hipEventCreate(&h->evf1)); HIPCHK(hipEventCreate(&h->evf2));
     }
+    int least = 0, greatest = 0;
+    HIPCHK(hipDeviceGetStreamPriorityRange(&least, &greatest));
+    const int asked = h->tune.region_priority;
+    h->prio_inert = (asked == 1 && least == 0) || (asked == 2 && greatest == 0);
+    h->prio_form = h->prio_inert ? 0 : asked;
+    h->lane_prio = h->prio_form == 1 ? least : 0;
+    h->chain_prio = greatest;
+    if (pooled && sb.lane_prio != h->lane_prio)
+      for (hipStream_t *st : {&h->pipe_r, &h->pipe_i, &h->pipe_x}) if (*st) { (void)hipStreamDestroy(*st); *st = nullptr; }
   }
   h->BT = BT; h->ntiles = (int)((B + BT - 1) / BT);
   h->lds = h->global_xs ? lds_bytes(0, BT, h->threads) : lds_bytes(an.Next + 2 * an.dt.k, BT, h->threads);
@@ -1272,6 +1287,8 @@
   bool open = false;
   int iter = 0, n_chunks = 0, n_lanes = 1;
   bool tail = false;
+  int chk_threads = 0;
+  bool lane_checks = false;
   double host_s = 0.0;
   std::vector<int> work, wl, tiles;
   std::vector<int> lane_last;
@@ -1312,14 +1329,20 @@
   const double t_begin = now_s();
   const int BT = h->BT, nq = (int)work.size();
   int rc;
-  if (!h->pipe_r) HIPCHK(hipStreamCreateWithFlags(&h->pipe_r, hipStreamNonBlocking));
-  if (!h->pipe_i) HIPCHK(hipStreamCreateWithFlags(&h->pipe_i, hipStreamNonBlocking));
+  auto lane_stream = [&](hipStream_t *st) -> int {
+    if (*st) return 0;
+    if (h->lane_prio != 0) HIPCHK(hipStreamCreateWithPriority(st, hipStreamNonBlocking, h->lane_prio));
+    else HIPCHK(hipStreamCreateWithFlags(st, hipStreamNonBlocking));
+    return 0;
+  };
+  if ((rc = lane_stream(&h->pipe_r)) || (rc = lane_stream(&h->pipe_i))) return rc;
   for (int k = 0; k < kPipeEvents; k++) if (!h->pipe_ev[k]) HIPCHK(hipEventCreate(&h->pipe_ev[k]));
-  hipEvent_t ev_fork = h->pipe_ev[0], ev_i0 = h->pipe_ev[1], ev_join = h->pipe_ev[2];
+  hipEvent_t ev_fork = h->pipe_ev[0], ev_i0 = h->pipe_ev[1], ev_join = h->pipe_ev[2], ev_chain = h->pipe_ev[kPipeEvents - 1];
   auto ev_chunk = [&](int c, int k) { return h->pipe_ev[3 + 3 * (c - 1) + k]; };
   auto ev_lane = [&](int l) { return h->pipe_ev[3 + 3 * kPipeChunks + l]; };
-  int n_even = h->tune.pipeline_chunks > 0 ? h->tune.pipeline_chunks : (nq + h->n_cus - 1) / h->n_cus;
-  int chunk_qps = (nq + n_even - 1) / n_even;
+  const int cus = h->tune.assume_cus > 0 ? std::min(h->n_cus, h->tune.assume_cus) : h->n_cus;
+  int chunk_qps = region_chunk_qps(nq, ra ? (int)ra->work.size() : 0, cus, kPipeChunks);
+  if (h->tune.pipeline_chunks > 0) chunk_qps = (nq + h->tune.pipeline_chunks - 1) / h->tune.pipeline_chunks;
   if (h->tune.pipeline_chunks <= 0 && h->tune.pipeline_chunk_qps > 0) chunk_qps = h->tune.pipeline_chunk_qps;
   const RefactorChunks ch = refactor_chunks(work, active, BT, chunk_qps, kPipeChunks);
   const int kbt = nq <= h->n_cus ? 1 : BT;
@@ -1327,8 +1350,11 @@
   const RefactorLanes rl = refactor_lanes(ch, work, BT, kbt, std::min(lanes_asked, kPipeLanes), h->tune.lanes_chunk0 < 0 ? kDefaultChunk0First : h->tune.lanes_chunk0 != 0,
                                           h->ntiles * BT + 4);
   const int L = rl.n_lanes;
-  if (L > 2 && !h->pipe_x) HIPCHK(hipStreamCreateWithFlags(&h->pipe_x, hipStreamNonBlocking));
+  if (L > 2 && (rc = lane_stream(&h->pipe_x))) return rc;
   if (ra && (L > 2 || BT != 1)) { g_last_error = "run-ahead beside three chunk lanes / tiles of several QPs"; return MI_OSQP_ERR_INVALID_SETTINGS; }
+  const bool chain_high = ra && h->prio_form == 2;
+  if (chain_high && !h->pipe_c) HIPCHK(hipStreamCreateWithPriority(&h->pipe_c, hipStreamNonBlocking, h->chain_prio));
+  const bool lane_checks = h->tune.lane_checks && BT == 1;
   std::vector<int> &wl = pr->wl;
   std::vector<int> wl_begin(1, 0);
   wl.clear();
@@ -1367,6 +1393,7 @@
       da.wg_base = base;
       HIPCHK(launch_tail(da, slots, h->dt_lds_asm, h->dt_lds, st));
     }
+    if (lane_checks) HIPCHK(launch_fail_flagged(a, wc, slots, BT, a.iter_begin, st));
     HIPCHK(hipEventRecord(ev_chunk(c, 2), st));
     return 0;
   };
@@ -1378,9 +1405,11 @@
     ai.rf_form = iterate_form(nt, h->rf_off != 0, h->tune);
     h->rf_launches[ai.rf_form]++;
     HIPCHK(launch_iterate(ai, BT, nt, h->threads, h->lds_iter + h->lds_factor, st));
+    if (lane_checks) HIPCHK(launch_check(ai, BT, nt, pr->chk_threads, h->lds, st));
     return 0;
   };
-  hipStream_t sx = h->stream;
+  hipStream_t sx = chain_high ? h->pipe_c : h->stream;
+  if (chain_high) HIPCHK(hipStreamWaitEvent(sx, ev_fork, 0));
   KernelArgs ac = a;
   ac.tiles = d_group; ac.res = nullptr; ac.info_at_end = 1;
   FactorArgs fg = make_factor_args(h, 0);
@@ -1442,11 +1471,14 @@
     for (int l = 0; l < L; l++) HIPCHK(hipEventRecord(ev_lane(l), lane[l]));
   }
   if (ra) for (size_t k = 1; k < ra->points.size(); k++) if ((rc = chain_segment(k))) return rc;
+  if (chain_high) { HIPCHK(hipEventRecord(ev_chain, sx)); HIPCHK(hipStreamWaitEvent(h->stream, ev_chain, 0)); }
   for (int l = 0; l < L; l++) HIPCHK(hipStreamWaitEvent(h->stream, ev_lane(l), 0));
   HIPCHK(hipEventRecord(ev_join, h->stream));
-  HIPCHK(launch_fail_flagged(a, h->work.p, (int)wl.size(), BT, a.iter_begin, h->stream));
-  pr->open = true; pr->iter = a.iter_begin; pr->n_chunks = ch.n_chunks; pr->n_lanes = L; pr->tail = tail;
+  if (!lane_checks) HIPCHK(launch_fail_flagged(a, h->work.p, (int)wl.size(), BT, a.iter_begin, h->stream));
+  pr->open = true; pr->iter = a.iter_begin; pr->n_chunks = ch.n_chunks; pr->n_lanes = L; pr->tail = tail; pr->lane_checks = lane_checks;
   h->refactor_lanes = std::max<int64_t>(h->refactor_lanes, L);
+  h->region_priority = h->prio_inert ? -1 : h->prio_form;
+  h->region_lane_checks = lane_checks; h->region_chunks = ch.n_chunks - 1;
   return 0;
 }
 
@@ -1540,7 +1572,7 @@
           HIPCHK(launch_iterate(a, BT, n_launch, h->mw_groups > 0 ? h->mw_threads : h->threads, h->lds_iter + h->lds_factor, h->stream));
           HIPCHK(hipEventRecord(h->ev1, h->stream));
         }
-        HIPCHK(launch_check(a, BT, n_launch, check_threads(), h->lds, h->stream));
+        if (!(iterated && region.open && region.lane_checks)) HIPCHK(launch_check(a, BT, n_launch, check_threads(), h->lds, h->stream));
         HIPCHK(hipMemcpyAsync(h->h_iscal, h->iscal.p, (size_t)ntl * IS_COUNT * BT * sizeof(int), hipMemcpyDeviceToHost, h->stream));
         if (a.res && !ra.used && is_rho_point(seg_end) && seg_end < S.max_iter) {
           HIPCHK(hipMemcpyAsync(h->h_res, h->ra_res.p, (size_t)2 * ntl * sizeof(double), hipMemcpyDeviceToHost, h->stream));
@@ -1601,6 +1633,7 @@
           KernelArgs nx = a;
           nx.iter_begin = iter; nx.iter_end = segment_end(iter); nx.info_at_end = 1;
           std::vector<int> work_m, active_m;
+          region.chk_threads = check_threads();
           if (a.res && !ra.used && res_iter == iter) {
             std::vector<double> pri(active.size()), dua(active.size());
             for (size_t i = 0; i < active.size(); i++) { pri[i] = h->h_res[2 * (size_t)active[i]]; dua[i] = h->h_res[2 * (size_t)active[i] + 1]; }
@@ -1672,6 +1705,7 @@
     if (h->pipe_r) (void)hipStreamSynchronize(h->pipe_r);
     if (h->pipe_i) (void)hipStreamSynchronize(h->pipe_i);
     if (h->pipe_x) (void)hipStreamSynchronize(h->pipe_x);
+    if (h->pipe_c) (void)hipStreamSynchronize(h->pipe_c);
     (void)hipStreamSynchronize(h->stream);
     return rc;
   }
@@ -1946,6 +1980,7 @@
   st->iterate_launches_long_head = h->rf_launches[RF_FORM_LONG_HEAD];
   st->runahead_regions = h->ra_regions; st->runahead_tiles = h->ra_tiles;
   st->runahead_left = h->ra_left; st->runahead_missed = h->ra_missed;
+  st->region_priority = h->region_priority; st->region_lane_checks = h->region_lane_checks; st->region_chunks = h->region_chunks;
   return MI_OSQP_OK;
 }
 
@@ -3627,6 +3662,13 @@
   std::copy(ch.tile_begin.begin(), ch.tile_begin.end(), tile_begin);
   return MI_OSQP_OK;
 }
+int mi_osqp_debug_region_chunks(int64_t nq, int64_t gw, int64_t n_cus, int64_t *chunk_qps, int64_t *n_chunks) {
+  if (!chunk_qps || !n_chunks) return MI_OSQP_ERR_NULL;
+  if (nq < 0 || nq > INT32_MAX || gw < 0 || gw > INT32_MAX || n_cus < 1 || n_cus > INT32_MAX) return MI_OSQP_ERR_INVALID_DATA;
+  const int q = region_chunk_qps((int)nq, (int)gw, (int)n_cus, streampool::kPipeChunks);
+  *chunk_qps = q; *n_chunks = (nq + q - 1) / q;
+  return MI_OSQP_OK;
+}
 int mi_osqp_debug_refactor_lanes(int64_t n_flagged, const int64_t *flagged, int64_t n_active, const int64_t *active, int64_t tile,
                                  int64_t chunk_qps, int64_t max_chunks, int64_t kbt, int64_t lanes, int64_t chunk0_first,
                                  int64_t scratch_slots, int64_t *n_lanes, int64_t *lane_of, int64_t *order, int64_t *order_begin,
```

After: 45900 (median of 6 runs). +6.7%, better.
